# lh3/bfc

Hardware: AMD Instinct MI355X
Metric: M k-mers/s counted (bloom+htab) on 150 bp reads (higher is better)
Workload: dtype u64

## Files before the change

bfc_amd/_lib.py:

```python
import ctypes as C
import os

HERE = os.path.dirname(os.path.abspath(__file__))
SO = os.environ.get("BFC_GPU_LIB") or os.path.join(HERE, "libbfc_gpu.so")

u64p = C.POINTER(C.c_uint64)
u32p = C.POINTER(C.c_uint32)
f32p = C.POINTER(C.c_float)


class BfcOpt(C.Structure):
    _fields_ = [("chunk_size", C.c_int), ("n_threads", C.c_int), ("no_mt_io", C.c_int), ("q", C.c_int), ("k", C.c_int),
                ("filter_mode", C.c_int), ("refine_ec", C.c_int), ("no_qual", C.c_int), ("min_frac", C.c_float),
                ("l_pre", C.c_int), ("bf_shift", C.c_int), ("n_hashes", C.c_int), ("discard", C.c_int),
                ("max_end_ext", C.c_int), ("win_multi_ec", C.c_int), ("min_cov", C.c_int),
                ("w_ec", C.c_int), ("w_ec_high", C.c_int), ("w_absent", C.c_int), ("w_absent_high", C.c_int),
                ("max_path_diff", C.c_int), ("max_heap", C.c_int)]


class BfcBf(C.Structure):
    _fields_ = [("n_shift", C.c_int), ("n_hashes", C.c_int), ("b", C.POINTER(C.c_uint8))]


class BfcKmer(C.Structure):
# ... 41 lines not shown
    "bfcg_mg_scatter": (C.c_int, [C.c_void_p, C.c_void_p, C.c_void_p, C.c_uint64, C.c_void_p, u32p]),
    "bfcg_mg_process": (C.c_int, [C.c_void_p, C.c_void_p, u32p]),
    "bfcg_mg_allow_onepass": (None, [C.c_void_p, C.c_int]),
    "bfcg_group_unique_id": (C.c_int, [C.c_void_p]),
    "bfcg_group_create": (C.c_void_p, [C.POINTER(BfcgParams), C.c_int, C.c_int, C.c_int, C.POINTER(C.c_int), C.c_void_p, C.c_int]),
    "bfcg_group_destroy": (None, [C.c_void_p]),
    "bfcg_group_info": (C.c_int, [C.c_void_p, C.POINTER(C.c_int)]),
    "bfcg_group_slab_mode": (C.c_int, [C.c_void_p]),
    "bfcg_group_lazy_batches": (C.c_uint64, [C.c_void_p]),
    "bfcg_group_exchange_bytes": (C.c_int, [C.c_void_p, u64p]),
    "bfcg_group_ctx": (C.c_void_p, [C.c_void_p, C.c_int]),
    "bfcg_group_reset": (C.c_int, [C.c_void_p]),
    "bfcg_group_count_batch_dev": (C.c_int, [C.c_void_p, C.POINTER(C.c_void_p), C.POINTER(C.c_void_p), u64p]),
    "bfcg_group_count_batch_host": (C.c_int, [C.c_void_p, C.c_void_p, C.c_void_p, C.c_uint64]),
    "bfcg_group_sync": (C.c_int, [C.c_void_p]),
    "bfcg_group_stats": (C.c_int, [C.c_void_p, u64p]),
    "bfcg_group_progress": (C.c_int, [C.c_void_p, u64p, u64p, u64p, C.c_int]),
    "bfcg_group_export_table": (C.c_void_p, [C.c_void_p]),
    "bfcg_group_export_bloom": (C.POINTER(BfcBf), [C.c_void_p, C.c_int]),
    "bfcg_group_export_bloom_resident": (C.POINTER(BfcBf), [C.c_void_p, C.c_int]),
    "bfcg_trim_create": (C.c_void_p, [C.c_int, C.POINTER(BfcBf), C.c_int, C.c_uint64, C.c_uint64]),
    "bfcg_trim_destroy": (None, [C.c_void_p]),
    "bfcg_trim_batch": (C.c_int, [C.c_void_p, C.c_void_p, C.c_void_p, C.c_uint64, u64p, C.c_uint64, C.c_float, C.POINTER(C.c_int32), C.POINTER(C.c_int32)]),
    "bfcg_trim_last_ms": (C.c_float, [C.c_void_p]),
    "bfcg_trim_adopted": (C.c_int, [C.c_void_p]),
    "bfcg_trim_dev_seq": (C.c_void_p, [C.c_void_p]),
    "bfcg_stream_batches": (C.c_uint64, [C.c_void_p]),
    "bfc_ch_union": (C.c_void_p, [C.POINTER(C.c_void_p), C.c_int]),
    "bfc_ingest_digest": (C.c_int, [C.c_char_p, C.c_uint64, C.c_uint64, C.c_int, u64p]),
    "bfc_ingest_planes_digest": (C.c_int, [C.c_char_p, C.c_uint64, C.c_uint64, C.c_int, C.c_int, C.c_int, u64p]),
    "bfc_pgz_digest": (C.c_int, [C.c_char_p, C.c_int, C.c_uint64, C.c_uint64, u64p]),
    "bfcg_kcov_create": (C.c_void_p, [C.c_void_p, C.c_int, C.c_uint64]),
    "bfcg_kcov_attach": (C.c_void_p, [C.c_void_p, C.c_uint64]),
    "bfcg_kcov_destroy": (None, [C.c_void_p]),
    "bfcg_kcov_batch": (C.c_int, [C.c_void_p, C.c_void_p, C.c_void_p, C.c_uint64, C.c_int, C.c_void_p]),
    "bfcg_kcov_last_ms": (C.c_float, [C.c_void_p]),
    "bfcg_kcov_dev_seq": (C.c_void_p, [C.c_void_p]),
    "bfcg_kcov_dev_out": (C.c_void_p, [C.c_void_p]),
    "bfcg_dev_alloc": (C.c_void_p, [C.c_void_p, C.c_uint64]),
    "bfcg_dev_free": (None, [C.c_void_p, C.c_void_p]),
    "bfcg_h2d": (C.c_int, [C.c_void_p, C.c_void_p, C.c_void_p, C.c_uint64]),
    "bfcg_d2h": (C.c_int, [C.c_void_p, C.c_void_p, C.c_void_p, C.c_uint64]),
    "bfcg_host_alloc": (C.c_void_p, [C.c_uint64]),
    "bfcg_host_free": (None, [C.c_void_p]),
    "bfcg_stats": (C.c_int, [C.c_void_p, u64p]),
    "bfcg_progress": (C.c_int, [C.c_void_p, u64p, u64p, u64p, C.c_int]),
    "bfcg_partition_info": (C.c_int, [C.c_void_p, u64p]),
    "bfcg_s1wc_launches": (C.c_uint64, []),
    "bfcg_table_info": (C.c_int, [C.c_void_p, C.POINTER(C.c_int)]),
    "bfcg_last_batch_ms": (C.c_int, [C.c_void_p, f32p]),
    "bfcg_stage_ms": (C.c_int, [C.c_void_p, C.POINTER(C.c_double), u64p, C.c_int]),
    "bfcg_bloom_to_host": (C.c_int, [C.c_void_p, C.c_int, C.c_void_p]),
    "bfcg_export_bloom": (C.POINTER(BfcBf), [C.c_void_p, C.c_int]),
    "bfcg_export_bloom_resident": (C.POINTER(BfcBf), [C.c_void_p, C.c_int]),
    "bfcg_resident_drop": (None, [C.c_void_p]),
    "bfcg_export_table": (C.c_void_p, [C.c_void_p]),
    "bfcg_export_table_resident": (C.c_void_p, [C.c_void_p]),
    "bfc_ch_get_lpre": (C.c_int, [C.c_void_p]),
    "bfc_ch_export_sorted": (C.c_uint64, [C.c_void_p, u32p, u64p]),
    "bfcg_ec_create": (C.c_void_p, [C.c_void_p, C.POINTER(BfcOpt), C.c_int, C.c_uint64, C.c_uint64]),
    "bfcg_ec_attach": (C.c_void_p, [C.c_void_p, C.POINTER(BfcOpt), C.c_uint64, C.c_uint64]),
    "bfcg_ec_batch": (C.c_int, [C.c_void_p, C.c_void_p, C.c_void_p, C.c_uint64, u64p, C.c_uint64, u32p, u32p]),
    "bfcg_ec_destroy": (None, [C.c_void_p]),
    "bfcg_ec_last_ms": (C.c_float, [C.c_void_p]),
    "bfcg_ec_host_reads": (C.c_uint64, [C.c_void_p]),
    "bfcg_ec_last_lookups": (C.c_uint64, [C.c_void_p]),
    "bfcg_ec_retry_reads": (C.c_uint64, [C.c_void_p]),
    "bfcg_ec_adopted": (C.c_int, [C.c_void_p]),
    "bfcg_ec1_host": (C.c_int, [C.c_void_p, C.POINTER(BfcOpt), C.c_int, C.c_void_p, C.c_void_p, u32p, u32p]),
    "bfcg_ec_batch_refine": (C.c_int, [C.c_void_p, C.c_void_p, C.c_void_p, C.c_uint64, u64p, C.c_uint64, u32p, u32p, u32p, u32p]),
    "bfcg_ec1_host_refine": (C.c_int, [C.c_void_p, C.POINTER(BfcOpt), C.c_int, C.c_void_p, C.c_void_p, C.c_uint32, C.c_uint32, u32p, u32p]),
    "bfcg_ec_parse_stats": (C.c_int, [C.c_char_p, u32p, u32p]),
    "bfcg_kmers_create": (C.c_void_p, [C.c_void_p, C.c_int]),
    "bfcg_kmers_attach": (C.c_void_p, [C.c_void_p]),
    "bfcg_kmers_destroy": (None, [C.c_void_p]),
    "bfcg_kmers_info": (C.c_int, [C.c_void_p, C.POINTER(C.c_int)]),
    "bfcg_kmers_hist": (C.c_int, [C.c_void_p, u64p, u64p]),
    "bfcg_kmers_sub_sizes": (C.c_int, [C.c_void_p, u32p]),
    "bfcg_kmers_hist_sizes": (C.c_int, [C.c_void_p, u64p, u64p, u32p]),
    "bfcg_kmers_list": (C.c_int, [C.c_void_p, C.c_int, C.c_int, C.c_uint32, C.c_uint32, C.c_void_p, C.c_void_p, C.c_uint64, u64p]),
    "bfcg_kmers_last_ms": (C.c_float, [C.c_void_p]),
    "bfcg_kmer_decode_host": (C.c_int, [C.c_int, C.c_int, C.c_uint32, C.c_uint64, u64p]),
    "bfcg_kmer_2str": (None, [C.c_int, u64p, C.c_char_p]),
    "bfcg_kmers_format": (C.c_uint64, [C.c_int, C.c_void_p, C.c_void_p, C.c_uint64, C.c_void_p]),
    "bfcg_kmers_format_sizes": (C.c_uint64, [C.c_void_p, C.c_uint64, C.c_void_p]),
    "bfcg_kmers_lookup": (C.c_int, [C.c_void_p, C.c_void_p, C.c_uint64, C.c_void_p, u64p]),
    "bfcg_kmers_profile": (C.c_int, [C.c_void_p, C.c_void_p, C.c_void_p, C.c_uint64, C.c_void_p]),
    "bfcg_kmer_from_str": (C.c_int, [C.c_int, C.c_char_p, u64p]),
    "bfcg_kmer_occ_host": (C.c_int, [C.c_void_p, u64p]),
    "bfcg_kmers_occ_host": (None, [C.c_void_p, C.c_void_p, C.c_uint64, C.c_void_p]),
    "bfcg_kmers_parse": (C.c_uint64, [C.c_int, C.c_char_p, C.c_uint64, C.c_void_p, C.c_uint64, u64p]),
    "bfcg_lookup_format": (C.c_uint64, [C.c_char_p, C.c_uint64, C.c_void_p, C.c_uint64, C.c_void_p]),
    "bfcg_profile_format": (C.c_uint64, [C.c_void_p, C.c_uint64, C.c_void_p]),
    "bfcg_kmers_read_stats": (C.c_int, [C.c_void_p, C.c_void_p, C.c_void_p, C.c_uint64, C.c_void_p, C.c_uint64, C.c_int, C.c_void_p]),
    "bfcg_read_stats_host": (C.c_int, [C.c_void_p, C.c_void_p, C.c_uint64, C.c_void_p, C.c_uint64, C.c_int, C.c_void_p]),
    "bfcg_read_stats_format": (C.c_uint64, [C.c_void_p, C.c_uint64, C.c_void_p]),
    "bfcg_hash_positions": (C.c_int, [C.c_void_p, C.c_void_p, C.c_void_p, C.c_uint64, u64p]),
    "bfcg_seen_flags": (C.c_int, [C.c_void_p, C.c_void_p, C.c_uint64]),
}

_lib = None


def load():
    global _lib
    if _lib is None:
        if not os.path.exists(SO):
            raise OSError("libbfc_gpu.so is not built (run `python -m bfc_amd.build`); there is no fallback path")
        L = C.CDLL(SO)
        for name, (res, args) in SYMBOLS.items():
            f = getattr(L, name)
            f.restype = res
            f.argtypes = args
        _lib = L
    return _lib


def build_id():
    return load().bfcg_build_id().decode()


def check_build_id():
    from . import build
    have, want = build_id(), "src:" + build.source_hash()
    if not have.startswith(want):
        raise OSError("libbfc_gpu.so is stale: built from %s, the tree is %s (run `python -m bfc_amd.build`)" % (have, want))
    return have
```

bfc_amd/api.py:

```python
import ctypes as C
import math

import numpy as np

from . import _lib
from ._lib import BfcOpt, BfcgParams, BfcKmer, u64p, u32p, f32p

STAT_NAMES = {0: "n_kmers", 1: "n_high", 2: "n_seen", 3: "n_keys", 4: "tab_ovf", 5: "err_pool", 6: "slow_buckets", 7: "crowded_regions", 8: "tab_cshift", 9: "n_batches"}


class BfcGpuError(RuntimeError):
    pass


def bfc_opt_init():
    o = BfcOpt()
    o.chunk_size = 100000000
    o.n_threads = 1
    o.q = 20
    o.k = 33
    o.l_pre = 20
    o.bf_shift = 33
    o.n_hashes = 4
    o.min_frac = 0.9
# ... 217 lines not shown
        self = cls.__new__(cls)
        self.L = _lib.load()
        self.ctx, self.params, self._borrowed = ctx, params, True
        self.rank, self.n_ranks, self.bf_shift, self.k = 0, n_ranks, params.bf_shift, params.k
        return self

    def _ck(self, rc):
        if rc != 0:
            raise BfcGpuError(self.L.bfcg_last_error().decode())

    def close(self):
        if self.ctx and not getattr(self, "_borrowed", False):
            self.L.bfcg_destroy(self.ctx)
        self.ctx = None

    def __del__(self):
        try:
            self.close()
        except Exception:
            pass

    def reset(self):
        self._ck(self.L.bfcg_reset(self.ctx))

    def count_host(self, seq_stream, qual_stream=None):
        seq_stream = np.ascontiguousarray(seq_stream, dtype=np.uint8)
        q = np.ascontiguousarray(qual_stream, dtype=np.uint8) if qual_stream is not None else None
        self._ck(self.L.bfcg_count_batch_host(self.ctx, seq_stream.ctypes.data, q.ctypes.data if q is not None else None, len(seq_stream)))

    def count_planes(self, planes, first_pos, n_pos, has_qual=True):
        planes = np.ascontiguousarray(planes, dtype=np.uint32)
        assert planes.ndim == 2 and planes.shape[0] == 4
        self._ck(self.L.bfcg_count_batch_planes(self.ctx, planes.ctypes.data, planes.shape[1], first_pos, n_pos, 1 if has_qual else 0))

    def count_dev(self, d_seq, d_qual, n_pos):
        self._ck(self.L.bfcg_count_batch_dev(self.ctx, d_seq, d_qual, n_pos))

    def mg_info(self):
        out = (C.c_int * 4)()
        self.L.bfcg_mg_info(self.ctx, out)
        return dict(nb1=out[0], nb_loc=out[1], rec_bytes=out[2], n_ranks=out[3])

    def batch_limit(self):
        return int(self.L.bfcg_batch_limit(self.ctx))

    def mg_scatter(self, d_seq, d_qual, n_pos, d_send):
        counts = np.zeros(self.mg_info()["nb1"], dtype=np.uint32)
        self._ck(self.L.bfcg_mg_scatter(self.ctx, d_seq, d_qual, n_pos, d_send, counts.ctypes.data_as(u32p)))
        return counts

    def mg_process(self, d_recv, seg_cnt):
        seg_cnt = np.ascontiguousarray(seg_cnt, dtype=np.uint32)
        self._ck(self.L.bfcg_mg_process(self.ctx, d_recv, seg_cnt.ctypes.data_as(u32p)))

    def dev_alloc(self, nbytes):
        p = self.L.bfcg_dev_alloc(self.ctx, nbytes)
        if not p:
            raise BfcGpuError(self.L.bfcg_last_error().decode())
        return p

    def dev_free(self, p):
        self.L.bfcg_dev_free(self.ctx, p)

    def h2d(self, dptr, arr):
        arr = np.ascontiguousarray(arr)
        self._ck(self.L.bfcg_h2d(self.ctx, dptr, arr.ctypes.data, arr.nbytes))

    def sync(self):
        self._ck(self.L.bfcg_sync(self.ctx))

    def stats(self):
        out = np.zeros(16, dtype=np.uint64)
        self._ck(self.L.bfcg_stats(self.ctx, out.ctypes.data_as(u64p)))
        d = {STAT_NAMES[i]: int(out[i]) for i in STAT_NAMES}
        d["stream_batches"] = int(self.L.bfcg_stream_batches(self.ctx))
        d["phase_cycles"] = [int(out[i]) for i in range(10, 16)]
        return d

    def table_info(self):
        out = (C.c_int * 4)()
        self.L.bfcg_table_info(self.ctx, out)
        return dict(segments=bool(out[0]), seg_shift=out[1], tab_cshift=out[2], seg_growths=out[3])

    def partition_info(self):
        out = (C.c_uint64 * 2)()
        self.L.bfcg_partition_info(self.ctx, out)
        return dict(one_pass=bool(out[0] & 1), level2_one_pass=bool(out[0] & 2), replayed_batches=int(out[1]))

    def s1wc_launches(self):
        return int(self.L.bfcg_s1wc_launches())

    def last_batch_ms(self):
        out = np.zeros(6, dtype=np.float32)
        self.L.bfcg_last_batch_ms(self.ctx, out.ctypes.data_as(f32p))
        return dict(hist1=float(out[0]), scatter1=float(out[1]), level2=float(out[2]), bloom=float(out[3]), commit=float(out[4]), total=float(out[5]))

    def stage_ms(self, reset=False):
        out = (C.c_double * 6)()
        n = C.c_uint64()
        self._ck(self.L.bfcg_stage_ms(self.ctx, out, C.byref(n), int(reset)))
        return dict(hist1=out[0], scatter1=out[1], level2=out[2], bloom=out[3], commit=out[4], total=out[5]), int(n.value)

    def bloom_bytes(self, which=0):
        out = np.empty((1 << (self.bf_shift - 3)) // self.n_ranks, dtype=np.uint8)
        self._ck(self.L.bfcg_bloom_to_host(self.ctx, which, out.ctypes.data))
        return out

    def export_bloom(self, which=0, resident=False):
        p = (self.L.bfcg_export_bloom_resident if resident else self.L.bfcg_export_bloom)(self.ctx, which)
        if not p:
            raise BfcGpuError(self.L.bfcg_last_error().decode())
        return HostBloom(p)

    def export_table(self):
        p = self.L.bfcg_export_table(self.ctx)
        if not p:
            raise BfcGpuError(self.L.bfcg_last_error().decode())
        return HostTable(p)

    def hash_positions(self, seq_stream, qual_stream=None):
        seq_stream = np.ascontiguousarray(seq_stream, dtype=np.uint8)
        q = np.ascontiguousarray(qual_stream, dtype=np.uint8) if qual_stream is not None else None
        out = np.zeros((len(seq_stream), 3), dtype=np.uint64)
        self._ck(self.L.bfcg_hash_positions(self.ctx, seq_stream.ctypes.data, q.ctypes.data if q is not None else None, len(seq_stream), out.ctypes.data_as(u64p)))
        return out

    def seen_flags(self, n_pos):
        out = np.zeros(n_pos, dtype=np.uint8)
        self._ck(self.L.bfcg_seen_flags(self.ctx, out.ctypes.data, n_pos))
        return out


class GpuGroup:

    def __init__(self, k, bf_shift, devices, max_batch_pos, n_ranks=None, first_rank=0, uid=None, transport=0, q=20, n_hashes=4, l_pre=20,
                 filter_mode=0, track_order=False, table_layout=0, region_shift=0, tab_cshift=0):
        self.L = _lib.load()
        p = BfcgParams()
        self.L.bfcg_params_default(C.byref(p))
        p.k, p.q, p.bf_shift, p.n_hashes, p.l_pre, p.filter_mode = k, q, bf_shift, n_hashes, l_pre, filter_mode
        p.max_batch_pos, p.region_shift, p.tab_cshift, p.track_order, p.table_layout = int(max_batch_pos), region_shift, tab_cshift, int(track_order), int(table_layout)
        self.params, self.k, self.bf_shift = p, k, bf_shift
        self.devices = list(devices)
        self.n_local = len(self.devices)
        self.n_ranks = n_ranks if n_ranks is not None else self.n_local
        dv = (C.c_int * self.n_local)(*self.devices)
        self._uid = (C.c_uint8 * 128).from_buffer_copy(bytes(uid)) if uid is not None else None
        self.g = self.L.bfcg_group_create(C.byref(p), self.n_ranks, first_rank, self.n_local, dv, self._uid, transport)
        if not self.g:
            raise BfcGpuError("bfcg_group_create failed: " + self.L.bfcg_last_error().decode())

    @staticmethod
    def unique_id():
        L = _lib.load()
        buf = (C.c_uint8 * 128)()
        if L.bfcg_group_unique_id(buf) != 0:
            raise BfcGpuError(L.bfcg_last_error().decode())
        return bytes(buf)

    def _ck(self, rc):
        if rc != 0:
            raise BfcGpuError(self.L.bfcg_last_error().decode())

    def close(self):
        if self.g:
            self.L.bfcg_group_destroy(self.g)
            self.g = None

    def __del__(self):
        try:
# ... 417 lines not shown
```

bfc_amd/csrc/bfcg_bloom3.hip:

```cpp
#include <hip/hip_runtime.h>
#include <stdint.h>
#include <stdlib.h>
#include "kmer_dev.h"
#include "bfcg_internal.h"
#include "bfcg_dev.h"

using namespace bfcg;

#define B3_UND 0x40000000u
#define B3_SEEN 0x40000000u
#define B3_COLD_NR 8
template <int BT, int PF, bool COLD>
__global__ __launch_bounds__(BT, PF <= 2 ? 8 : 6) void k_bloom3(KParams P, BloomArgs A)
{
	extern __shared__ __attribute__((aligned(16))) unsigned char smem[];
	__shared__ uint32_t s_list_n, s_ovf, s_pool_off, s_emit_n, s_fs_used, s_wb_n, s_pad3[2];
	const uint32_t f = blockIdx.x;
	const bool ho_log = A.ho_stride != 0;
	if (batch_poisoned(A)) { if (ho_log && threadIdx.x == 0) A.ho_mark[f] = A.ho_cur[f]; return; }
	uint32_t rs, n;
	region_list(A, f, rs, n);
	if (n == 0) { if (threadIdx.x == 0) { if (ho_log) A.ho_mark[f] = A.ho_cur[f]; else if (A.agg_cnt) A.agg_cnt[f] = 0; } return; }
	uint32_t ho_cur0 = 0;
	unsigned long long *ho_base;
	if (ho_log) {
		ho_cur0 = A.ho_cur[f];
		if (ho_cur0 + n > A.ho_stride) {
			if (threadIdx.x == 0) { atomicAdd(&A.stats[(size_t)(f & (ST_SLOTS - 1)) * ST_N + ST_ERR_POOL], 1ULL); A.ho_mark[f] = ho_cur0; }
			return;
		}
		ho_base = A.ho + (uint64_t)f * A.ho_stride + ho_cur0;
	} else ho_base = reinterpret_cast<unsigned long long *>(A.stream_out) + rs;
	A.stats += (size_t)(f & (ST_SLOTS - 1)) * ST_N;
	const uint32_t region_dw = 16u << P.R;
	unsigned char *sp = smem;
	unsigned int *region = reinterpret_cast<unsigned int *>(sp); sp += (size_t)region_dw * 4;
	const uint32_t nblk = 1u << P.R;
	unsigned int *bcnt = reinterpret_cast<unsigned int *>(sp), *boff = bcnt + nblk;
	if (COLD) sp += (size_t)(2 * nblk + 4) * 4;
	unsigned int *fs = reinterpret_cast<unsigned int *>(sp); if (!COLD) sp += (size_t)P.fs_cap * 4;
	unsigned int *la = reinterpret_cast<unsigned int *>(sp); sp += (size_t)P.list_cap * 4;
	unsigned int *lb = reinterpret_cast<unsigned int *>(sp); sp += (size_t)P.list_cap * 4;
	unsigned short *lc = reinterpret_cast<unsigned short *>(sp); sp += (size_t)P.list_cap * 2;
	unsigned short *ord = reinterpret_cast<unsigned short *>(sp);
	const uint32_t fs_mask = P.fs_cap - 1;
	const uint32_t *recs = A.recs + (uint64_t)rs * 3;
	unsigned int *g_region = reinterpret_cast<unsigned int *>(A.bloom) + (uint64_t)f * region_dw;
	const uint32_t imp = (P.f_base + f) >> P.F2;
	const Dec3 D = dec3_geom(P);
	const int tid = threadIdx.x, lane = tid & 63;
	const uint32_t mask_a = (1u << D.a) - 1u, imp_sh = D.n ? imp << D.lo : 0u, sh_up = D.lo + D.n;
#ifdef BFCG_MEASURE
	const bool timing = BFCG_ABL(P, 64) && tid == 0;
	long long tq[7] = {0, 0, 0, 0, 0, 0, 0};
	if (timing) tq[0] = clock64();
#endif
	auto addr3 = [&](uint32_t d0, uint32_t d1) -> uint32_t {
		const uint32_t y0d = d0 & mask_a, upper = y0d >> D.up;
		const uint32_t y0lo = D.n ? (y0d & D.lowmask) | imp_sh | (upper << sh_up) : y0d;
		const uint32_t y1lo = __builtin_amdgcn_alignbit(d1, d0, D.a) & D.mk32;
		const uint32_t hh = upper | (((y0lo - y1lo) ^ y1lo) << D.sh_x);
		uint32_t h2 = (hh >> 9) & 511u;
		h2 |= (uint32_t)((h2 & 31u) == 0);
		return (y0d & D.rmask) | ((hh & 511u) << 8) | (h2 << 17);
	};
	auto entry3 = [&](uint32_t d0, uint32_t d1) -> unsigned long long {
		const unsigned long long AA = d0 | ((unsigned long long)d1 << 32);
		const unsigned long long y1 = (AA >> D.a) & ((1ULL << P.k) - 1);
		const uint32_t y0d = d0 & mask_a;
		const unsigned long long id = (unsigned long long)((y0d & D.rmask) | ((y0d >> D.up) << D.R)) | (y1 << D.sh_y1);
		return (id << 1) | (unsigned long long)((d1 >> D.sh_flag) & 1u);
	};
	RecW<3> cur[PF], nxt[PF];
#pragma unroll
	for (int u = 0; u < PF; ++u) {
		const uint32_t i = tid + u * BT;
		cur[u].d[0] = cur[u].d[1] = cur[u].d[2] = 0; nxt[u] = cur[u];
		if (i < n) cur[u] = rec_load<3>(recs + (uint64_t)i * 3);
		if (i + BT * PF < n) nxt[u] = rec_load<3>(recs + (uint64_t)(i + BT * PF) * 3);
	}
	{
		const uint4 *src = reinterpret_cast<const uint4 *>(g_region);
		uint4 *dst = reinterpret_cast<uint4 *>(region);
		for (uint32_t i = tid; i < region_dw / 4; i += BT) dst[i] = src[i];
		if constexpr (COLD) { for (uint32_t i = tid; i < 2 * nblk + 4; i += BT) bcnt[i] = 0; }
		else {
			uint4 *f4 = reinterpret_cast<uint4 *>(fs);
			for (uint32_t i = tid; i < P.fs_cap / 4; i += BT) f4[i] = make_uint4(FS32_EMPTY, FS32_EMPTY, FS32_EMPTY, FS32_EMPTY);
		}
		if (tid == 0) { s_list_n = 0; s_emit_n = 0; s_ovf = 0; s_fs_used = 0; s_wb_n = 0; }
	}
	__syncthreads();
#ifdef BFCG_MEASURE
	if (timing) tq[1] = clock64();
#endif
	volatile uint32_t *v_ovf = &s_ovf;

	for (uint32_t base = 0; base < n; base += BT * PF) {
		uint32_t pk[PF], um[PF];
#pragma unroll
		for (int u = 0; u < PF; ++u) {
			pk[u] = 0; um[u] = 0;
			if (base + u * BT + (uint32_t)(tid & ~63) < n) {
				pk[u] = addr3(cur[u].d[0], cur[u].d[1]);
				const B3Pos b = b3_positions((pk[u] >> 8) & 511u, pk[u] >> 17);
				const uint32_t bl64 = (pk[u] & 255u) << 6;
				const uint32_t w0 = *b3_wordp(region, bl64, b.b0), w1 = *b3_wordp(region, bl64, b.b1), w2 = *b3_wordp(region, bl64, b.b2), w3 = *b3_wordp(region, bl64, b.b3);
				um[u] = (b3_bit(w0, b.b0) | (b3_bit(w1, b.b1) << 1) | (b3_bit(w2, b.b2) << 2) | (b3_bit(w3, b.b3) << 3)) ^ 15u;
			}
		}
		unsigned long long ms[PF], ml[PF];
		uint32_t tot_s = 0, tot_l = 0;
#pragma unroll
		for (int u = 0; u < PF; ++u) {
			const bool act = base + tid + u * BT < n;
			ms[u] = __ballot(act && um[u] == 0); ml[u] = __ballot(act && um[u] != 0);
			tot_s += (uint32_t)__popcll(ms[u]); tot_l += (uint32_t)__popcll(ml[u]);
		}
		uint32_t o_s = 0, o_l = 0;
		if (lane == 0) { if (tot_s) o_s = atomicAdd(&s_emit_n, tot_s); if (tot_l) o_l = atomicAdd(&s_list_n, tot_l); }
		o_s = __builtin_amdgcn_readfirstlane(o_s); o_l = __builtin_amdgcn_readfirstlane(o_l);
#pragma unroll
		for (int u = 0; u < PF; ++u) {
			const uint32_t below_lo = (uint32_t)__builtin_amdgcn_mbcnt_lo((uint32_t)ms[u], 0u), below_s = (uint32_t)__builtin_amdgcn_mbcnt_hi((uint32_t)(ms[u] >> 32), below_lo);
			const uint32_t blow_lo = (uint32_t)__builtin_amdgcn_mbcnt_lo((uint32_t)ml[u], 0u), below_l = (uint32_t)__builtin_amdgcn_mbcnt_hi((uint32_t)(ml[u] >> 32), blow_lo);
			const bool act = base + tid + u * BT < n;
			if (act && um[u] == 0) {
				ho_base[o_s + below_s] = entry3(cur[u].d[0], cur[u].d[1]);
				if (A.seen_out) A.seen_out[cur[u].d[2]] = 2;
			} else if (act) {
				const uint32_t li = o_l + below_l;
				if (li < P.list_cap) {
					la[li] = cur[u].d[2]; lb[li] = pk[u] | (um[u] << 26); lc[li] = (unsigned short)(base + tid + u * BT);
					if constexpr (COLD) __hip_atomic_fetch_add(&bcnt[pk[u] & 255u], 1u, __ATOMIC_RELAXED, __HIP_MEMORY_SCOPE_WORKGROUP);
				}
			}
			o_s += (uint32_t)__popcll(ms[u]); o_l += (uint32_t)__popcll(ml[u]);
		}
		if (base + BT * PF < n) {
#pragma unroll
			for (int u = 0; u < PF; ++u) {
				cur[u] = nxt[u];
				const uint32_t i = base + 2 * BT * PF + tid + u * BT;
				if (i < n) nxt[u] = rec_load<3>(recs + (uint64_t)i * 3);
			}
		}
	}
	__syncthreads();
#ifdef BFCG_MEASURE
	if (timing) tq[2] = clock64();
#endif
	const uint32_t ln = s_list_n;
	const bool ovf_list = ln > P.list_cap || ln > (COLD ? (uint32_t)(B3_COLD_NR * BT) : 8191u) || n > 65535u;
	bool dirty = true;
	if constexpr (COLD) {
		if (!ovf_list) {
			if (tid < 64) {
				const uint32_t per = (nblk + 63u) >> 6, b0 = (uint32_t)tid * per;
				uint32_t v[4] = {0, 0, 0, 0}, sum = 0;
#pragma unroll
				for (int t = 0; t < 4; ++t) if ((uint32_t)t < per && b0 + t < nblk) { v[t] = bcnt[b0 + t]; sum += v[t]; }
				uint32_t inc = sum;
#pragma unroll
				for (int o = 1; o < 64; o <<= 1) { const uint32_t x = __shfl_up(inc, o); if (lane >= o) inc += x; }
				uint32_t run = inc - sum;
#pragma unroll
				for (int t = 0; t < 4; ++t) if ((uint32_t)t < per && b0 + t < nblk) { boff[b0 + t] = run; bcnt[b0 + t] = run; run += v[t]; }
				if (tid == 63) boff[nblk] = inc;
			}
			__syncthreads();
			for (uint32_t li = tid; li < ln; li += BT) ord[atomicAdd(&bcnt[lb[li] & 255u], 1u)] = (unsigned short)li;
			__syncthreads();
			uint32_t mv[B3_COLD_NR];
#pragma unroll
			for (int t = 0; t < B3_COLD_NR; ++t) {
				const uint32_t pos = (uint32_t)tid + (uint32_t)t * BT;
				mv[t] = 0;
				if (pos < ln) {
					const uint32_t li = ord[pos], x = la[li], bl = lb[li] & 255u, s0 = boff[bl], s1 = boff[bl + 1];
					uint32_t r = 0;
					for (uint32_t j = s0; j < s1; ++j) r += (uint32_t)(la[ord[j]] < x);
					mv[t] = ((s0 + r) << 16) | li;
				}
			}
			__syncthreads();
#pragma unroll
			for (int t = 0; t < B3_COLD_NR; ++t) { const uint32_t pos = (uint32_t)tid + (uint32_t)t * BT; if (pos < ln) ord[mv[t] >> 16] = (unsigned short)mv[t]; }
			__syncthreads();
			if ((uint32_t)tid < nblk) {
				const uint32_t bl = (uint32_t)tid, bl64 = bl << 6, s0 = boff[bl], s1 = boff[bl + 1];
				uint32_t li_n = s0 < s1 ? ord[s0] : 0u, w_n = s0 < s1 ? lb[li_n] : 0u;
				for (uint32_t j = s0; j < s1; ++j) {
					const uint32_t li = li_n, w = w_n;
					if (j + 1 < s1) { li_n = ord[j + 1]; w_n = lb[li_n]; }
					const B3Pos b = b3_positions((w >> 8) & 511u, (w >> 17) & 511u);
					unsigned int *p0 = b3_wordp(region, bl64, b.b0), *p1 = b3_wordp(region, bl64, b.b1), *p2 = b3_wordp(region, bl64, b.b2), *p3 = b3_wordp(region, bl64, b.b3);
					const uint32_t w0 = *p0, w1 = *p1, w2 = *p2, w3 = *p3;
					const uint32_t clr = (b3_bit(w0, b.b0) | (b3_bit(w1, b.b1) << 1) | (b3_bit(w2, b.b2) << 2) | (b3_bit(w3, b.b3) << 3)) ^ 15u;
					if (clr == 0) lb[li] = w | B3_SEEN;
					else {
						if (clr & 1u) __hip_atomic_fetch_or(p0, 1u << (b.b0 & 31u), __ATOMIC_RELAXED, __HIP_MEMORY_SCOPE_WORKGROUP);
						if (clr & 2u) __hip_atomic_fetch_or(p1, 1u << (b.b1 & 31u), __ATOMIC_RELAXED, __HIP_MEMORY_SCOPE_WORKGROUP);
						if (clr & 4u) __hip_atomic_fetch_or(p2, 1u << (b.b2 & 31u), __ATOMIC_RELAXED, __HIP_MEMORY_SCOPE_WORKGROUP);
						if (clr & 8u) __hip_atomic_fetch_or(p3, 1u << (b.b3 & 31u), __ATOMIC_RELAXED, __HIP_MEMORY_SCOPE_WORKGROUP);
					}
				}
			}
			__syncthreads();
			for (uint32_t t0 = 0; t0 < ln; t0 += BT) {
				const uint32_t li = t0 + tid;
				bool seen = false;
				if (li < ln) {
					seen = (lb[li] & B3_SEEN) != 0;
					if (A.seen_out) A.seen_out[la[li]] = seen ? 2 : 1;
				}
				const unsigned long long vote = __ballot(seen);
				if (vote) {
					uint32_t o = 0;
					if (lane == 0) o = atomicAdd(&s_emit_n, (uint32_t)__popcll(vote));
					o = __builtin_amdgcn_readfirstlane(o);
					if (seen) {
						const RecW<3> r = rec_load<3>(recs + (uint64_t)lc[li] * 3);
						ho_base[o + (uint32_t)__builtin_amdgcn_mbcnt_hi((uint32_t)(vote >> 32), __builtin_amdgcn_mbcnt_lo((uint32_t)vote, 0u))] = entry3(r.d[0], r.d[1]);
					}
				}
			}
			dirty = ln != 0;
			__syncthreads();
		}
	} else
	if (!ovf_list) {
		for (uint32_t li = tid; li < ln; li += BT) {
			const uint32_t w = lb[li], bl = w & 255u, bl64 = bl << 6, um = (w >> 26) & 15u;
			const B3Pos b = b3_positions((w >> 8) & 511u, (w >> 17) & 511u);
			uint32_t o0 = 0, o1 = 0, o2 = 0, o3 = 0;
			if (um & 1u) o0 = atomicOr(b3_wordp(region, bl64, b.b0), 1u << (b.b0 & 31u));
			if (um & 2u) o1 = atomicOr(b3_wordp(region, bl64, b.b1), 1u << (b.b1 & 31u));
			if (um & 4u) o2 = atomicOr(b3_wordp(region, bl64, b.b2), 1u << (b.b2 & 31u));
			if (um & 8u) o3 = atomicOr(b3_wordp(region, bl64, b.b3), 1u << (b.b3 & 31u));
			uint32_t cm = (b3_bit(o0, b.b0) | (b3_bit(o1, b.b1) << 1) | (b3_bit(o2, b.b2) << 2) | (b3_bit(o3, b.b3) << 3)) & um;
			if (cm) {
				*(volatile uint32_t *)&s_fs_used = 1;
				__hip_atomic_fetch_or(&region[bl * 16u], 1u, __ATOMIC_RELAXED, __HIP_MEMORY_SCOPE_WORKGROUP);
				const uint32_t idx = la[li];
				const uint32_t p01 = b.b0 | (b.b1 << 16), p23 = b.b2 | (b.b3 << 16);
				while (cm) {
					const int j = __ffs((int)cm) - 1;
					cm &= cm - 1;
					const uint32_t bj = ((j & 2 ? p23 : p01) >> ((j & 1) << 4)) & 0xffffu;
					if (!fs32_insert(fs, fs_mask, bl * 512u + bj, li, idx, la)) *v_ovf = 1;
				}
			}
		}
	}
	__syncthreads();
#ifdef BFCG_MEASURE
	if (timing) tq[6] = clock64();
#endif
	const bool ovf = ovf_list || s_ovf;
	if (COLD && !ovf) ;
	else if (!ovf) {
		if (s_fs_used) {
			auto compete_entry = [&](uint32_t li) {
				const uint32_t w = lb[li], bl = w & 255u, um = (w >> 26) & 15u;
				const B3Pos b = b3_positions((w >> 8) & 511u, (w >> 17) & 511u);
				const uint32_t q0 = bl * 512u + b.b0, q1 = bl * 512u + b.b1, q2 = bl * 512u + b.b2, q3 = bl * 512u + b.b3;
				const uint32_t c0 = fs[fs32_slot(q0, fs_mask)], c1 = fs[fs32_slot(q1, fs_mask)], c2 = fs[fs32_slot(q2, fs_mask)], c3 = fs[fs32_slot(q3, fs_mask)];
				uint32_t todo = ((uint32_t)(c0 != FS32_EMPTY) | ((uint32_t)(c1 != FS32_EMPTY) << 1) | ((uint32_t)(c2 != FS32_EMPTY) << 2) | ((uint32_t)(c3 != FS32_EMPTY) << 3)) & um;
				bool und = todo == um;
				if (todo) {
					const uint32_t idx = la[li];
					const uint32_t p01 = b.b0 | (b.b1 << 16), p23 = b.b2 | (b.b3 << 16);
					while (todo) {
						const int j = __ffs((int)todo) - 1;
						todo &= todo - 1;
						const uint32_t bj = ((j & 2 ? p23 : p01) >> ((j & 1) << 4)) & 0xffffu;
						und &= fs32_compete(fs, fs_mask, bl * 512u + bj, li, idx, la);
					}
				}
				if (und) lb[li] = w | B3_UND;
			};
			unsigned short *const wb = lc + ln;
			const uint32_t wb_cap = P.list_cap - ln;
			for (uint32_t li0 = 0; li0 < ln; li0 += BT) {
				const uint32_t li = li0 + tid;
				bool want = false;
				if (li < ln) {
					want = (region[(lb[li] & 255u) * 16u] & 1u) != 0;
					if (!want && A.seen_out) A.seen_out[la[li]] = 1;
				}
				const unsigned long long vote = __ballot(want);
				if (vote) {
					uint32_t o = 0;
					if (lane == 0) o = atomicAdd(&s_wb_n, (uint32_t)__popcll(vote));
					o = __builtin_amdgcn_readfirstlane(o);
					if (want) {
						const uint32_t slot = o + (uint32_t)__builtin_amdgcn_mbcnt_hi((uint32_t)(vote >> 32), __builtin_amdgcn_mbcnt_lo((uint32_t)vote, 0u));
						if (slot < wb_cap) wb[slot] = (unsigned short)li;
						else compete_entry(li);
					}
				}
			}
			__syncthreads();
			const uint32_t wb_all = s_wb_n, wb_n = wb_all < wb_cap ? wb_all : wb_cap;
			for (uint32_t t = tid; t < wb_n; t += BT) compete_entry(wb[t]);
			__syncthreads();
			const bool wl_ok = wb_all <= wb_cap;
			const uint32_t cn = wl_ok ? wb_n : ln;
			for (uint32_t t0 = 0; t0 < cn; t0 += BT) {
				const uint32_t t = t0 + tid;
				uint32_t li = 0;
				bool seen = false;
				if (t < cn) {
					li = wl_ok ? (uint32_t)wb[t] : t;
					const uint32_t w = lb[li];
					if (w & B3_UND) {
						const uint32_t bl = w & 255u, um = (w >> 26) & 15u;
						const B3Pos b = b3_positions((w >> 8) & 511u, (w >> 17) & 511u);
						bool first = false;
						if (um & 1u) first |= fs32_lookup(fs, fs_mask, bl * 512u + b.b0) == li;
						if (um & 2u) first |= fs32_lookup(fs, fs_mask, bl * 512u + b.b1) == li;
						if (um & 4u) first |= fs32_lookup(fs, fs_mask, bl * 512u + b.b2) == li;
						if (um & 8u) first |= fs32_lookup(fs, fs_mask, bl * 512u + b.b3) == li;
						seen = !first;
					}
					if (A.seen_out) A.seen_out[la[li]] = seen ? 2 : 1;
				}
				const unsigned long long vote = __ballot(seen);
				if (vote) {
					uint32_t o = 0;
					if (lane == 0) o = atomicAdd(&s_emit_n, (uint32_t)__popcll(vote));
					o = __builtin_amdgcn_readfirstlane(o);
					if (seen) {
						const RecW<3> r = rec_load<3>(recs + (uint64_t)lc[li] * 3);
						ho_base[o + (uint32_t)__popcll(vote & ((1ULL << lane) - 1))] = entry3(r.d[0], r.d[1]);
					}
				}
			}
			for (uint32_t i = tid; i < (1u << P.R); i += BT) region[i * 16u] &= ~0xffu;
		} else if (A.seen_out) {
			for (uint32_t li = tid; li < ln; li += BT) A.seen_out[la[li]] = 1;
		}
		dirty = ln != 0;
		__syncthreads();
	} else {
		const int nh = 4;
		uint64_t want = (uint64_t)n * nh * 2;
		const uint64_t lim = (uint64_t)(1u << P.R) * 512 * 2;
		if (want > lim) want = lim;
		uint32_t cap = 1024; while (cap < want) cap <<= 1;
		if (tid == 0) {
			uint32_t sl = f & (A.pool_slices - 1);
			while (atomicCAS(&A.pool[sl], 0ULL, 1ULL) != 0ULL) sl = (sl + 1) & (A.pool_slices - 1);
			s_pool_off = sl; s_emit_n = 0;
			atomicAdd(&A.stats[ST_SLOW_BUCKETS], 1ULL);
		}
		{
			const uint4 *src = reinterpret_cast<const uint4 *>(g_region);
			uint4 *dst = reinterpret_cast<uint4 *>(region);
			for (uint32_t i = tid; i < region_dw / 4; i += BT) dst[i] = src[i];
		}
		__syncthreads();
		unsigned long long *gfs = A.pool + A.pool_slices + (uint64_t)s_pool_off * lim;
		for (uint32_t i = tid; i < cap; i += BT) gfs[i] = FS_EMPTY;
		__threadfence();
		__syncthreads();
		const uint32_t gmask = cap - 1;
		for (uint32_t i = tid; i < n; i += BT) {
			const RecW<3> r = rec_load<3>(recs + (uint64_t)i * 3);
			const uint32_t w = addr3(r.d[0], r.d[1]), bl = w & 255u;
			uint32_t z = (w >> 8) & 511u;
			for (int j = 0; j < nh; ++j) {
				const uint32_t b = bloom_next(z, w >> 17);
				if (!b3_bit(*b3_wordp(region, bl << 6, b), b)) fs_insert<true>(gfs, gmask, bl * 512 + b, r.d[2], gmask);
			}
		}
		__threadfence();
		__syncthreads();
		for (uint32_t i0 = 0; i0 < n; i0 += BT) {
			const uint32_t i = i0 + tid;
			bool seen = false;
			RecW<3> r; r.d[0] = r.d[1] = r.d[2] = 0;
			if (i < n) {
				r = rec_load<3>(recs + (uint64_t)i * 3);
				const uint32_t w = addr3(r.d[0], r.d[1]), bl = w & 255u;
				uint32_t z = (w >> 8) & 511u; bool first = false, unresolved = false;
				for (int j = 0; j < nh; ++j) {
					uint32_t b = bloom_next(z, w >> 17), fi;
					if (fs_lookup<true>(gfs, gmask, bl * 512 + b, fi)) {
						unresolved = true; first |= (fi == r.d[2]);
						atomicOr(b3_wordp(region, bl << 6, b), 1u << (b & 31));
					}
				}
				seen = !unresolved || !first;
				if (A.seen_out) A.seen_out[r.d[2]] = seen ? 2 : 1;
			}
			const unsigned long long vote = __ballot(seen);
			if (vote) {
				uint32_t o = 0;
				if (lane == 0) o = atomicAdd(&s_emit_n, (uint32_t)__popcll(vote));
				o = __builtin_amdgcn_readfirstlane(o);
				if (seen) ho_base[o + (uint32_t)__popcll(vote & ((1ULL << lane) - 1))] = entry3(r.d[0], r.d[1]);
			}
		}
		__syncthreads();
		if (tid == 0) { __threadfence(); atomicExch(&A.pool[s_pool_off], 0ULL); }
	}
#ifdef BFCG_MEASURE
	if (timing) tq[3] = clock64();
#endif
	if (dirty) {
		uint4 *dst = reinterpret_cast<uint4 *>(g_region);
		const uint4 *src = reinterpret_cast<const uint4 *>(region);
		for (uint32_t i = tid; i < region_dw / 4; i += BT) dst[i] = src[i];
	}
#ifdef BFCG_MEASURE
	if (timing) tq[4] = clock64();
#endif
	if (tid == 0) {
		const uint32_t ns = s_emit_n;
		if (ns) atomicAdd(&A.stats[ST_SEEN], (unsigned long long)ns);
		if (ho_log) { A.ho_cur[f] = ho_cur0 + ns; A.ho_mark[f] = ho_cur0 + ns; }
		else if (A.agg_cnt) A.agg_cnt[f] = ns;
	}
#ifdef BFCG_MEASURE
	if (timing) {
		tq[5] = clock64();
		for (int t = 0; t < 5; ++t) atomicAdd(&A.stats[10 + t], (unsigned long long)(tq[t + 1] - tq[t]));
		atomicAdd(&A.stats[15], (unsigned long long)(tq[6] - tq[2]));
	}
#endif
	(void)s_pad3;
}

namespace bfcg {

typedef void (*BloomFn)(KParams, BloomArgs);
static BloomFn bloom3_kernel(bool pf2, bool cold)
{
	if (cold) return pf2 ? k_bloom3<512, 2, true> : k_bloom3<512, 4, true>;
	return pf2 ? k_bloom3<512, 2, false> : k_bloom3<512, 4, false>;
}
static hipError_t set_bloom3_max_lds(BloomFn fn, int lds) { return hipFuncSetAttribute((const void *)fn, hipFuncAttributeMaxDynamicSharedMemorySize, lds < BLOOM3_LDS_FLOOR ? BLOOM3_LDS_FLOOR : lds); }
hipError_t set_bloom3_lds_attr(int lds)
{
	hipError_t e = hipSuccess;
	for (int i = 0; i < 4 && e == hipSuccess; ++i) e = set_bloom3_max_lds(bloom3_kernel(i & 1, i & 2), lds);
	return e;
}

void run_bloom3(const KParams &P, const BloomArgs &A, int nfine, size_t lds, hipStream_t st)
{
	static int pf = 0;
	if (!pf) { const char *e = getenv("BFCG_B3_PF"); pf = e && atoi(e) == 2 ? 2 : e && atoi(e) == 4 ? 4 : 1; }
	const bool pf2 = P.b3_cold ? P.b3_warm != 0 : pf == 2 || (pf == 1 && P.b3_warm);
	hipLaunchKernelGGL(bloom3_kernel(pf2, P.b3_cold != 0), dim3(nfine), dim3(512), lds, st, P, A);
}

}

struct Dec4 { int up, iw, is; uint32_t rmask; };
__device__ __forceinline__ Dec4 dec4_geom(const KParams &P)
{
	Dec4 g;
	g.up = P.rec_n ? P.rec_lo : P.bf_shift - 9;
	const int io = (P.k - P.rec_n) + P.k + 1;
	g.iw = io >> 5; g.is = io & 31; g.rmask = (1u << P.R) - 1u;
	return g;
}
template <int BT, int PF>
__global__ __launch_bounds__(BT, 6) void k_bloom3fm(KParams P, BloomArgs A)
{
	extern __shared__ __attribute__((aligned(16))) unsigned char smem[];
	__shared__ uint32_t s_list_n, s_seen;
	const uint32_t f = blockIdx.x;
	if (batch_poisoned(A)) return;
	uint32_t rs, n;
	region_list(A, f, rs, n);
	if (n == 0) return;
	A.stats += (size_t)(f & (ST_SLOTS - 1)) * ST_N;
	const uint32_t region_dw = 16u << P.R, nblk = 1u << P.R;
	unsigned char *sp = smem;
	unsigned int *region = reinterpret_cast<unsigned int *>(sp); sp += (size_t)region_dw * 4;
	unsigned int *region_hi = reinterpret_cast<unsigned int *>(sp); sp += (size_t)region_dw * 4;
	unsigned int *bcnt = reinterpret_cast<unsigned int *>(sp), *boff = bcnt + nblk; sp += (size_t)(2 * nblk + 4) * 4;
	unsigned int *la = reinterpret_cast<unsigned int *>(sp); sp += (size_t)P.list_cap * 4;
	unsigned int *lb = reinterpret_cast<unsigned int *>(sp); sp += (size_t)P.list_cap * 4;
	unsigned short *ord = reinterpret_cast<unsigned short *>(sp);
	const uint32_t *recs = A.recs + (uint64_t)rs * 4;
	unsigned int *g_region = reinterpret_cast<unsigned int *>(A.bloom) + (uint64_t)f * region_dw;
	unsigned int *g_region_hi = reinterpret_cast<unsigned int *>(A.bloom_hi) + (uint64_t)f * region_dw;
	const Dec4 D = dec4_geom(P);
	const int tid = threadIdx.x, lane = tid & 63;
	auto addr4 = [&](uint32_t d0, uint32_t d1) -> uint32_t {
		const uint32_t hh = __builtin_amdgcn_alignbit(d1, d0, D.up);
		uint32_t h2 = (hh >> 9) & 511u;
		h2 |= (uint32_t)((h2 & 31u) == 0);
		return (d0 & D.rmask) | ((hh & 511u) << 8) | (h2 << 17);
	};
	auto idx4 = [&](const RecW<4> &r) -> uint32_t {
		const uint32_t a = D.iw == 0 ? r.d[0] : D.iw == 1 ? r.d[1] : D.iw == 2 ? r.d[2] : r.d[3], b = D.iw == 0 ? r.d[1] : D.iw == 1 ? r.d[2] : r.d[3];
		return D.is ? __builtin_amdgcn_alignbit(b, a, D.is) : a;
	};
	auto set_hi = [&](uint32_t bl64, const B3Pos &b) {
		__hip_atomic_fetch_or(b3_wordp(region_hi, bl64, b.b0), 1u << (b.b0 & 31u), __ATOMIC_RELAXED, __HIP_MEMORY_SCOPE_WORKGROUP);
		__hip_atomic_fetch_or(b3_wordp(region_hi, bl64, b.b1), 1u << (b.b1 & 31u), __ATOMIC_RELAXED, __HIP_MEMORY_SCOPE_WORKGROUP);
		__hip_atomic_fetch_or(b3_wordp(region_hi, bl64, b.b2), 1u << (b.b2 & 31u), __ATOMIC_RELAXED, __HIP_MEMORY_SCOPE_WORKGROUP);
		__hip_atomic_fetch_or(b3_wordp(region_hi, bl64, b.b3), 1u << (b.b3 & 31u), __ATOMIC_RELAXED, __HIP_MEMORY_SCOPE_WORKGROUP);
	};
	{
		const uint4 *src = reinterpret_cast<const uint4 *>(g_region), *src2 = reinterpret_cast<const uint4 *>(g_region_hi);
		uint4 *dst = reinterpret_cast<uint4 *>(region), *dst2 = reinterpret_cast<uint4 *>(region_hi);
		for (uint32_t i = tid; i < region_dw / 4; i += BT) { dst[i] = src[i]; dst2[i] = src2[i]; }
	}
	uint32_t r = 0, sh = 32, seen_total = 0;
	bool dirty = false;
	const uint32_t cap = P.list_cap < (uint32_t)(B3_COLD_NR * BT) ? P.list_cap : (uint32_t)(B3_COLD_NR * BT);
	for (;;) {
		for (uint32_t i = tid; i < 2 * nblk + 4; i += BT) bcnt[i] = 0;
		if (tid == 0) { s_list_n = 0; s_seen = 0; }
		__syncthreads();
		uint32_t my_seen = 0;
		RecW<4> rec[PF], nxt[PF];
#pragma unroll
		for (int u = 0; u < PF; ++u) {
			const uint32_t i = tid + u * BT;
			rec[u].d[0] = rec[u].d[1] = rec[u].d[2] = rec[u].d[3] = 0; nxt[u] = rec[u];
			if (i < n) rec[u] = rec_load<4>(recs + (uint64_t)i * 4);
			if (i + BT * PF < n) nxt[u] = rec_load<4>(recs + (uint64_t)(i + BT * PF) * 4);
		}
		for (uint32_t base = 0; base < n; base += BT * PF) {
			uint32_t pk[PF], um[PF], ix[PF];
			bool act[PF];
#pragma unroll
			for (int u = 0; u < PF; ++u) {
				ix[u] = idx4(rec[u]);
				act[u] = base + tid + u * BT < n && (sh == 32 || (ix[u] >> sh) == r);
				pk[u] = addr4(rec[u].d[0], rec[u].d[1]);
				const B3Pos b = b3_positions((pk[u] >> 8) & 511u, pk[u] >> 17);
// ... 132 lines not shown
```

bfc_amd/csrc/bfcg_ctx.hip:

```cpp
#include <hip/hip_runtime.h>
#include <stdint.h>
#include <stdio.h>
#include <stdlib.h>
#include <string.h>
#include <stdarg.h>
#include <sys/mman.h>
#include <time.h>
#include <vector>
#include <thread>
#include "bfc_gpu.h"
#include "bfcg_internal.h"
#include "bfc_host.h"

using namespace bfcg;

static thread_local char g_err[512] = "";
enum { HO_MAX_PAGES = BFCG_HO_MAX_PAGES };
enum { OP_FLAG_WORDS = 12, OP_STICKY = 8 };
static double dbg_now(void) { struct timespec ts; clock_gettime(CLOCK_MONOTONIC, &ts); return ts.tv_sec + 1e-9 * ts.tv_nsec; }
static inline void set_seg_shift(KParams &P, int s, int blk_max) { P.seg_shift = s; P.seg_blk = s < blk_max ? s : blk_max; }
int bfcg::fail(const char *fmt, ...)
{
	va_list ap; va_start(ap, fmt); vsnprintf(g_err, sizeof(g_err), fmt, ap); va_end(ap);
	fprintf(stderr, "[E::bfcg] %s\n", g_err);
	return -1;
}

struct bfcg_ctx {
	bfcg_params_t prm;
	KParams P;
	BatchBufs B;
	hipStream_t st;
	hipStream_t stA;
	hipStream_t stC;
	hipEvent_t evt[2][7];
	hipEvent_t evA[2], evB[2], evCopy;
	uint32_t *rows1[2], *chunk1[2], *start1[2]; uint64_t *recs1[2];
	uint8_t *d_seq2[2], *d_qual2[2];
	uint32_t *d_planes[2];
	uint64_t plane_cap;
	int cur, pend;
	int used[2];
	uint8_t *d_seq, *d_qual;
	unsigned long long *h_stats;
	unsigned long long *h_snap[2];
	uint64_t call_no, slot_call[2];
	int call_depth;
	uint64_t final_call, call_keys[64];
	uint64_t n_batches;
	float last_ms[6];
	double sum_ms[6]; uint64_t n_timed;
	int rw;
	uint64_t bloom_bytes;
	int n_ranks, rank, log2n;
	uint32_t *d_seg, *h_seg;
	size_t seg_words;
	uint64_t recv_cap;
	uint64_t keys_last, grow[2];
	uint64_t crowded_last;
	int stream_mode;
	uint32_t *stream_out; uint64_t n_stream_batches;
	double seen_per_pos;
	int cold;
	uint64_t seen_last, pos_final, slot_pos[2];
	int pipeline;
	int seg_ok;
	int seg_total_max;
	int seg_blk_max;
	int b3_ok;
	uint32_t fs_cap_w, list_cap_w;
	uint32_t list_cap_cw;
	uint32_t list_cap_c;
	int seg_init_shift;
	int seg_escaped;
	uint64_t n_seg_grow;
	int onepass_ok, onepass;
	uint32_t *op_cursor[2], *op_seg[2], *op_flags, *h_flags[2];
	int unfinished, unfinished_mg;
	uint32_t *h_rows[2]; int rows_slot;
	uint32_t op_cap; uint64_t op_min_pos;
	uint32_t *cnt2; uint32_t cap2; uint64_t recs2_n;
	struct opq_t { const uint8_t *seq, *qual; uint64_t n_pos; int slot; const void *recv; int mg; } opq[4]; int n_opq;
	int mg_op2_ok, mg_op2, mg_op2_allowed; uint32_t *mg_seg[4];
	int mg_slab_ok; int mg_seg_slab[4];
	uint64_t n_replayed;
	int reused;
	int seg_no_grow;
	int seg_cap_shift;
	unsigned long long *ho, *ho_keys, *h_ho_keys[2]; uint32_t *ho_cur, *ho_mark; uint32_t ho_stride; int ho_K;
	int ho_pending;
	uint64_t ho_page_call[HO_MAX_PAGES];
	int slot_commit[2]; uint64_t slot_page_call[2][HO_MAX_PAGES];
	int slot_all_committed[2];
	uint64_t keys_known;
	int commit_absorbed;
	uint64_t keys_per_batch; int n_commits, ho_window;
	unsigned long long *seg_spare; int seg_spare_shift;
};

extern "C" const char *bfcg_last_error(void) { return g_err; }
extern "C" void bfcg_set_error(const char *msg) { fail("%s", msg); }

extern "C" int bfcg_device_count(void)
{
	int ndev = 0;
	if (hipGetDeviceCount(&ndev) != hipSuccess) { (void)hipGetLastError(); return 0; }
	return ndev;
}

extern "C" void bfcg_params_default(bfcg_params_t *p)
{
	memset(p, 0, sizeof(*p));
	p->k = 33; p->q = 20; p->bf_shift = 33; p->n_hashes = 4; p->l_pre = 20;
	p->max_batch_pos = 1ULL << 27;
}

static int clamp_lpre(int k, int l_pre)
{
	if (k * 2 - l_pre > BFC_CH_KEYBITS) l_pre = k * 2 - BFC_CH_KEYBITS;
	if (l_pre > BFC_CH_MAXPRE) l_pre = BFC_CH_MAXPRE;
	return l_pre;
}

extern "C" bfcg_ctx_t *bfcg_create(const bfcg_params_t *prm)
{
	int ndev = 0;
	const bool timing = getenv("BFC_GPU_TIMING") != 0;
	const double t_c0 = dbg_now();
	if (hipGetDeviceCount(&ndev) != hipSuccess || ndev == 0) { fail("no HIP device available: the counting path has no CPU fallback"); return NULL; }
	const double t_c1 = dbg_now();
	if (prm->device < 0 || prm->device >= ndev) { fail("device %d out of range (%d devices)", prm->device, ndev); return NULL; }
	if (prm->k < 1 || prm->k > 63) { fail("k=%d outside [1,63] (bfc.h:8, htab.c:23)", prm->k); return NULL; }
	if (prm->bf_shift < 9 + 0 || prm->bf_shift > 37) { fail("bf_shift=%d outside [9,37] (bbf.c:9, bfc.h:9)", prm->bf_shift); return NULL; }
	if (prm->n_hashes < 1 || prm->n_hashes > 12) { fail("n_hashes=%d outside [1,12]", prm->n_hashes); return NULL; }
	if (prm->max_batch_pos == 0 || prm->max_batch_pos >= (1ULL << 32)) { fail("max_batch_pos must be in [1, 2^32)"); return NULL; }
	const int n_ranks = prm->n_ranks > 0 ? prm->n_ranks : 1;
	int log2n = 0; while ((1 << log2n) < n_ranks) ++log2n;
	if ((1 << log2n) != n_ranks || n_ranks > 64 || prm->rank < 0 || prm->rank >= n_ranks) { fail("n_ranks=%d must be a power of two <= 64 and 0 <= rank=%d < n_ranks", n_ranks, prm->rank); return NULL; }
	if (n_ranks > 1 && prm->max_batch_pos >= (1ULL << (32 - log2n))) { fail("with %d ranks a batch holds < 2^%d positions", n_ranks, 32 - log2n); return NULL; }
	BFCG_CKN((void)0, hipSetDevice(prm->device));

	bfcg_ctx_t *c = (bfcg_ctx_t *)calloc(1, sizeof(bfcg_ctx_t));
	if (!c) { fail("out of host memory"); return NULL; }
	c->prm = *prm;
	KParams &P = c->P;
	P.k = prm->k; P.q = prm->q; P.bf_shift = prm->bf_shift; P.n_hashes = prm->n_hashes; P.filter_mode = prm->filter_mode;
	P.l_pre = clamp_lpre(prm->k, prm->l_pre);
	if (!prm->filter_mode && 2 * prm->k < P.l_pre) {
		fail("k=%d is too small for l_pre=%d: the count table needs 2k >= l_pre (htab.c:45-58)", prm->k, P.l_pre); bfcg_destroy(c); return NULL;
	}
	{
		const char *e;
		P.R = prm->region_shift > 0 ? prm->region_shift : ((e = getenv("BFCG_R")) ? atoi(e) : 8);
		if (P.R > 10) P.R = 10;
		if (P.R < 4) P.R = 4;
		if (P.R > P.bf_shift - 9) P.R = P.bf_shift - 9;
		while (P.bf_shift - 9 - P.R > 20 && P.R < 10) ++P.R;
		P.F = P.bf_shift - 9 - P.R;
		if (P.F <= 8) { P.F1 = P.F; P.F2 = 0; }
		else { P.F2 = (P.F + 1) / 2; if (P.F2 > 10) P.F2 = 10; P.F1 = P.F - P.F2; }
		if (P.F2 > 0 && (e = getenv("BFCG_F1"))) {
			const int f1 = atoi(e);
			if (f1 >= 1 && f1 <= 10 && P.F - f1 >= 1 && P.F - f1 <= 10 && f1 >= log2n) { P.F1 = f1; P.F2 = P.F - f1; }
		}
		if (P.F1 > 10) { fail("bf_shift=%d needs more than two scatter levels at region_shift=%d", P.bf_shift, P.R); bfcg_destroy(c); return NULL; }
		if (n_ranks > 1 && P.F2 == 0) {
			if (P.F <= log2n) { fail("bf_shift=%d gives %d bloom regions: too few for %d ranks", P.bf_shift, 1 << P.F, n_ranks); bfcg_destroy(c); return NULL; }
			P.F1 = (P.F + 1) / 2 > log2n ? (P.F + 1) / 2 : log2n; P.F2 = P.F - P.F1;
// ... 524 lines not shown
static int seg_maintain(bfcg_ctx_t *c)
{
	KParams &P = c->P; BatchBufs &B = c->B;
	const uint64_t nf = nfine(c);
	const double t_dbg = dbg_now();
	struct dbg_guard { double t; int s0; const int *s1; ~dbg_guard() { if (getenv("BFCG_DEBUG") && *s1 != s0) fprintf(stderr, "[D::seg_maintain] shift %d -> %d: %.3f ms\n", s0, *s1, (dbg_now() - t) * 1e3); } } dg{t_dbg, P.seg_shift, &P.seg_shift};
	for (;;) {
		const uint64_t ovf = c->h_stats[ST_TAB_OVF];
		const int target = seg_target_shift(c);
		if (ovf == 0 && target == P.seg_shift) return 0;
		if (ovf > B.tab_ovf_cap) return fail("count table overflow list exhausted (%llu parked k-mers)", (unsigned long long)ovf);
		{
			size_t free_b = 0, total_b = 0;
			const bool no_room = hipMemGetInfo(&free_b, &total_b) == hipSuccess && ((nf << target) * 8) + (1ULL << 30) > (uint64_t)free_b + (c->seg_spare && c->seg_spare_shift >= target ? (nf << c->seg_spare_shift) * 8 : 0);
			if (no_room || target > c->seg_total_max) {
				if (ovf == 0 && (double)c->h_stats[ST_KEYS] < 0.85 * (double)(nf << P.seg_shift)) { c->seg_no_grow = 1; return 0; }
				if (target > c->seg_total_max) return seg_to_legacy(c);
				if (seg_to_legacy(c) == 0) return 0;
				return fail("count table of %llu keys cannot grow to 2^%d slots per region: %.1f GiB of device memory free", (unsigned long long)c->h_stats[ST_KEYS], target, free_b / 1073741824.0);
			}
		}
		const int old_shift = P.seg_shift, old_blk = P.seg_blk;
		unsigned long long *nt = 0;
		int nt_shift = target;
		set_seg_shift(P, target, c->seg_blk_max);
		if (c->seg_spare && c->seg_spare_shift >= target) { nt = c->seg_spare; nt_shift = c->seg_spare_shift; c->seg_spare = 0; }
		else {
			if (c->seg_spare) { BFCG_CK(hipFree(c->seg_spare)); c->seg_spare = 0; }
			BFCG_CK(hipMalloc(&nt, (nf << target) * 8));
		}
		run_seg_rehash(P, B.seg_tab, old_shift, old_blk, nt, (uint32_t)nf, c->st);
		BFCG_CK(hipStreamSynchronize(c->st));
		BFCG_CK(hipGetLastError());
		if (((nf << nt_shift) * 8) <= (16ULL << 30)) {
			if (c->seg_cap_shift < nt_shift && c->reused) { BFCG_CK(hipFree(B.seg_tab)); c->seg_spare = 0; if (hipMalloc(&c->seg_spare, (nf << nt_shift) * 8) != hipSuccess) { (void)hipGetLastError(); c->seg_spare = 0; } c->seg_spare_shift = nt_shift; }
			else { c->seg_spare = B.seg_tab; c->seg_spare_shift = c->seg_cap_shift; }
		} else BFCG_CK(hipFree(B.seg_tab));
		B.seg_tab = nt; c->seg_cap_shift = nt_shift;
		++c->n_seg_grow;
		if (ovf) {
			uint64_t *tmp = 0;
			BFCG_CK(hipMalloc(&tmp, ovf * 40));
			BFCG_CK(hipMemcpyAsync(tmp, B.tab_ovf, ovf * 40, hipMemcpyDeviceToDevice, c->st));
			BFCG_CK(hipMemsetAsync(&B.stats[(size_t)ST_SLOTS * ST_N], 0, 8, c->st));
			run_seg_replay(P, B.seg_tab, tmp, ovf, B.stats, B.tab_ovf, B.tab_ovf_cap, c->st);
			if (fetch_stats(c) != 0) return -1;
			BFCG_CK(hipFree(tmp));
		} else c->h_stats[ST_TAB_OVF] = 0;
	}
}

static int seg_to_legacy(bfcg_ctx_t *c, int for_export)
{
	KParams &P = c->P; BatchBufs &B = c->B;
	const uint64_t nf = nfine(c);
	const uint64_t keys = c->h_stats[ST_KEYS];
	if (c->seg_spare) { BFCG_CK(hipFree(c->seg_spare)); c->seg_spare = 0; }
	if (!for_export && !P.filter_mode && !B.agg_out) BFCG_CK(hipMalloc(&B.agg_out, nf * P.ag_cap * (P.track ? 32 : 24)));
	int cs = c->prm.tab_cshift > 0 ? c->prm.tab_cshift : 2;
	const uint64_t want = for_export ? keys + keys * 3 / 4 : 2 * keys + (c->prm.max_batch_pos / 4);
	while ((1ULL << (P.l_pre + cs)) < want && P.l_pre + cs < 36) ++cs;
	{
		size_t free_b = 0, total_b = 0;
		if (hipMemGetInfo(&free_b, &total_b) == hipSuccess)
			while (cs > 1 && (8ULL << (P.l_pre + cs)) + (2ULL << 30) > (uint64_t)free_b) --cs;
	}
	P.tab_cshift = cs;
	BFCG_CK(hipMalloc(&B.table, 8ULL << (P.l_pre + cs)));
	BFCG_CK(hipMemsetAsync(B.table, 0, 8ULL << (P.l_pre + cs), c->st));
	BFCG_CK(hipMemset2DAsync(B.stats + ST_KEYS, sizeof(unsigned long long) * ST_N, 0, sizeof(unsigned long long), ST_SLOTS, c->st));
	run_seg_to_table(P, B.seg_tab, (uint32_t)nf, B.table, B.stats, B.tab_ovf, B.tab_ovf_cap, c->st);
	BFCG_CK(hipStreamSynchronize(c->st));
	BFCG_CK(hipGetLastError());
	BFCG_CK(hipFree(B.seg_tab));
	B.seg_tab = 0;
	P.seg = 0; P.b3 = 0; c->seg_escaped = 1;
	BFCG_CK(set_bloom_lds_attr(P));
	if (fetch_stats(c) != 0) return -1;
	c->keys_last = c->h_stats[ST_KEYS];
	if (for_export && c->h_stats[ST_TAB_OVF] == 0) return 0;
	return table_maintain(c);
}

extern "C" int bfcg_partition_info(bfcg_ctx_t *c, uint64_t out[2]) { out[0] = (uint64_t)((c->onepass ? 1 : 0) | ((c->onepass || (c->mg_op2 && c->mg_op2_allowed)) && c->cap2 ? 2 : 0)); out[1] = c->n_replayed; return 0; }
extern "C" void bfcg_mg_allow_onepass(bfcg_ctx_t *c, int on) { c->mg_op2_allowed = on != 0; }

extern "C" int bfcg_table_info(bfcg_ctx_t *c, int out[4])
{
	out[0] = c->P.seg; out[1] = c->P.seg ? c->P.seg_shift : 0; out[2] = c->P.seg ? 0 : c->P.tab_cshift; out[3] = (int)c->n_seg_grow;
	return 0;
}


static KParams batch_params(const bfcg_ctx_t *c, int no_kstats, int onepass1)
{
	KParams Pt = c->P;
	Pt.no_kstats = no_kstats;
	Pt.dedupe = dedupe_hint(c);
	warm_tables(c, Pt);
	if (onepass1) {
		const char *e = getenv("BFCG_L2_BIG");
		const int want = e ? atoi(e) : 0;
		Pt.l2_big = c->cap2 && want > 0 && Pt.F2 >= (want == 1 ? 9 : 10) && scatter2_big_ok(Pt);
	}
	return Pt;
}

static int batch_bufs(bfcg_ctx_t *c, BatchBufs &Bt)
{
	if (ensure_agg(c) != 0 || use_stream(c) != 0) return -1;
	Bt = c->B;
	Bt.batch_hi = (unsigned long long)(c->n_batches + 1) << 32;
	Bt.stream = c->stream_mode; Bt.stream_out = c->stream_out;
	return 0;
}

struct StageB {
	const uint64_t *in1; const uint32_t *seg_beg, *seg_end; int n_seg, segs_per_bucket; const uint32_t *row_base, *bucket_start; uint64_t rec_bound;
	int slabs;
	int queued;
	uint64_t call, pos;
	const uint8_t *seq, *qual;
	const void *recv; const uint32_t *sizes; int sizes_slab;
	int finalise;
};

static int opq_push(bfcg_ctx_t *c, int b, const StageB &w)
{
	if (c->n_opq == 4) return fail("internal: one-pass queue overflow");
	int mg = 0;
	if (w.recv) {
		const size_t words = (size_t)c->n_ranks * (size_t)((1 << c->P.F1) >> c->log2n) * (w.sizes_slab ? 8 : 1);
		for (;; ++mg) { int used = 0; for (int i = 0; i < c->n_opq; ++i) used |= c->opq[i].mg == mg + 1; if (!used) break; }
		if (w.sizes) memcpy(c->mg_seg[mg], w.sizes, sizeof(uint32_t) * words); else memset(c->mg_seg[mg], 0, sizeof(uint32_t) * words);
		c->mg_seg_slab[mg++] = w.sizes_slab;
	}
	c->opq[c->n_opq++] = bfcg_ctx::opq_t{w.seq, w.qual, w.pos, b, w.recv, mg};
	return 0;
}

static int enqueue_stage_b(bfcg_ctx_t *c, int b, BatchBufs &Bt, const KParams &Pt, const StageB &w)
{
	if (handover_begin(c, Bt, b, w.slabs, w.call) != 0) return -1;
	run_stage_b(Pt, Bt, w.in1, w.seg_beg, w.seg_end, w.n_seg, w.segs_per_bucket, w.row_base, w.bucket_start, w.rec_bound, c->st, c->evt[b]);
	if (handover_end(c, Bt, b) != 0) return -1;
	if (w.queued) {
		BFCG_CK(hipMemcpyAsync(c->h_flags[b] + 1, c->op_flags + OP_STICKY, sizeof(uint32_t), hipMemcpyDeviceToHost, c->st));
		if (opq_push(c, b, w) != 0) return -1;
	}
	BFCG_CK(hipMemcpyAsync(c->h_snap[b], c->B.stats, sizeof(unsigned long long) * ST_N * (ST_SLOTS + 1), hipMemcpyDeviceToHost, c->st));
	c->slot_call[b] = c->call_no = w.call; c->slot_pos[b] = w.pos;
	BFCG_CK(hipEventRecord(c->evB[b], c->st));
	BFCG_CK(hipGetLastError());
	c->used[b] = 1;
	++c->n_batches;
	return w.finalise ? finalise_previous(c, b) : 0;
}

static int mg_stage_b(bfcg_ctx_t *c, int b, const void *d_recv, const uint32_t *d, int n_seg, int spb, uint64_t rec_bound, const uint32_t *sizes, int sizes_slab, int finalise)
{
	BatchBufs Bt;
	if (batch_bufs(c, Bt) != 0) return -1;
	const int op2_run = c->mg_op2 && c->mg_op2_allowed && c->cap2;
	const int op2 = op2_run && rec_bound >= 8 * nfine(c);
	if (op2_run) Bt.op_sticky = c->op_flags + OP_STICKY;
	if (op2) {
		Bt.cnt2 = c->cnt2; Bt.cap2 = c->cap2; Bt.op_flags = c->op_flags + 4 * b;
		BFCG_CK(hipMemsetAsync(Bt.op_flags, 0, 4 * sizeof(uint32_t), c->st));
	}
	const StageB w = {(const uint64_t *)d_recv, d, d + n_seg, n_seg, spb, d + 2 * n_seg, d + 3 * n_seg + 1, rec_bound, op2, op2_run, c->call_no + 1, rec_bound, nullptr, nullptr, d_recv, sizes, sizes_slab, finalise};
	return enqueue_stage_b(c, b, Bt, batch_params(c, 0, 0), w);
}


extern "C" int bfcg_mg_info(bfcg_ctx_t *c, int out[4])
{
	out[0] = 1 << c->P.F1; out[1] = (1 << c->P.F1) >> c->log2n; out[2] = c->rw; out[3] = c->n_ranks;
	return 0;
}

static int mg_scatter2(bfcg_ctx_t *c, const uint8_t *d_seq, const uint8_t *d_qual, uint64_t n_pos, void *d_send, uint32_t *counts, int no_kstats);
extern "C" int bfcg_mg_scatter(bfcg_ctx_t *c, const uint8_t *d_seq, const uint8_t *d_qual, uint64_t n_pos, void *d_send, uint32_t *counts) { return mg_scatter2(c, d_seq, d_qual, n_pos, d_send, counts, 0); }
extern "C" int bfcg_mg_scatter_again(bfcg_ctx_t *c, const uint8_t *d_seq, const uint8_t *d_qual, uint64_t n_pos, void *d_send, uint32_t *counts) { return mg_scatter2(c, d_seq, d_qual, n_pos, d_send, counts, 1); }
static inline hipStream_t mg_stage_a_stream(bfcg_ctx_t *c) { return c->n_ranks == 1 && !c->pipeline ? c->st : c->stA; }
static int mg_stage_a_begin(bfcg_ctx_t *c, int b, hipStream_t sA, const uint8_t *d_seq, const uint8_t **d_qual, uint64_t n_pos)
{
	if (batch_fits(c, n_pos) != 0) return -1;
	BFCG_CK(hipSetDevice(c->prm.device));
	if (n_pos == 0) {
		for (int i = 0; i < 3; ++i) BFCG_CK(hipEventRecord(c->evt[b][i], sA));
		return 1;
	}
	return same_block_offset(c, b, d_seq, d_qual, n_pos, sA);
}
static BatchBufs mg_slab_bufs(const bfcg_ctx_t *c, int b, uint32_t own_delta)
{
	const uint32_t nb_loc = (1u << c->P.F1) >> c->log2n;
	BatchBufs Bt = c->B;
	Bt.op_cursor = c->op_cursor[b]; Bt.op_seg = c->op_seg[b]; Bt.op_flags = c->op_flags + 4 * b; Bt.op_cap = c->op_cap; Bt.cap2 = c->cap2;
	Bt.op_own_lo = (uint32_t)c->rank * nb_loc; Bt.op_own_n = nb_loc; Bt.op_own_delta = own_delta;
	return Bt;
}
static int mg_scatter2(bfcg_ctx_t *c, const uint8_t *d_seq, const uint8_t *d_qual, uint64_t n_pos, void *d_send, uint32_t *counts, int no_kstats)
{
	const int nb1 = 1 << c->P.F1, b = c->cur;
	const hipStream_t sA = mg_stage_a_stream(c);
	const int begun = mg_stage_a_begin(c, b, sA, d_seq, &d_qual, n_pos);
	if (begun == 1) memset(counts, 0, sizeof(uint32_t) * nb1);
	if (begun) return begun < 0 ? -1 : 0;
	BatchBufs Bt = c->B;
	Bt.rows1 = c->rows1[b]; Bt.chunk1 = c->chunk1[b]; Bt.start1 = c->start1[b]; Bt.row_base = Bt.start1 + nb1 + 1;
	KParams Pa = c->P;
	Pa.no_kstats = no_kstats;
	run_stage_a(Pa, Bt, d_seq, d_qual, (int64_t)n_pos, (uint64_t *)d_send, sA, c->evt[b]);
	BFCG_CK(hipGetLastError());
	uint32_t *tmp = (uint32_t *)malloc(sizeof(uint32_t) * (nb1 + 1));
	hipError_t e = hipMemcpyAsync(tmp, Bt.start1, sizeof(uint32_t) * (nb1 + 1), hipMemcpyDeviceToHost, sA);
	if (e == hipSuccess) e = hipStreamSynchronize(sA);
	if (e != hipSuccess) { free(tmp); return fail("reading the level-1 bucket starts failed: %s", hipGetErrorString(e)); }
	for (int i = 0; i < nb1; ++i) counts[i] = tmp[i + 1] - tmp[i];
	free(tmp);
	return 0;
}

extern "C" int bfcg_mg_slab_info(bfcg_ctx_t *c, uint32_t out[2]) { out[0] = c->op_cap; out[1] = (uint32_t)(c->mg_slab_ok && c->op_cursor[0] != 0); return 0; }
extern "C" int bfcg_mg_scatter_slabs(bfcg_ctx_t *c, const uint8_t *d_seq, const uint8_t *d_qual, uint64_t n_pos, void *d_send, uint32_t own_delta, uint32_t *fills, int *overflow)
// ... 648 lines not shown
```

bfc_amd/csrc/bfcg_dev.h:

```cpp
#pragma once
#include <hip/hip_runtime.h>
#include <stdint.h>
#include "kmer_dev.h"
#include "bfcg_internal.h"

using namespace bfcg;

template <int RD> struct RecW { uint32_t d[RD]; };

template <int RD> __device__ __forceinline__ RecW<RD> rec_load(const uint32_t *p);
template <> __device__ __forceinline__ RecW<3> rec_load<3>(const uint32_t *p)
{ const uint3 v = *reinterpret_cast<const uint3 *>(p); RecW<3> r; r.d[0] = v.x; r.d[1] = v.y; r.d[2] = v.z; return r; }
template <> __device__ __forceinline__ RecW<4> rec_load<4>(const uint32_t *p)
{ const uint4 v = *reinterpret_cast<const uint4 *>(p); RecW<4> r; r.d[0] = v.x; r.d[1] = v.y; r.d[2] = v.z; r.d[3] = v.w; return r; }
template <> __device__ __forceinline__ RecW<5> rec_load<5>(const uint32_t *p)
{ RecW<5> r; r.d[0] = p[0]; r.d[1] = p[1]; r.d[2] = p[2]; r.d[3] = p[3]; r.d[4] = p[4]; return r; }
template <int RD> __device__ __forceinline__ void rec_store(uint32_t *p, const RecW<RD> &r);
template <> __device__ __forceinline__ void rec_store<3>(uint32_t *p, const RecW<3> &r)
{ *reinterpret_cast<uint3 *>(p) = make_uint3(r.d[0], r.d[1], r.d[2]); }
template <> __device__ __forceinline__ void rec_store<4>(uint32_t *p, const RecW<4> &r)
{ *reinterpret_cast<uint4 *>(p) = make_uint4(r.d[0], r.d[1], r.d[2], r.d[3]); }
template <> __device__ __forceinline__ void rec_store<5>(uint32_t *p, const RecW<5> &r)
{ p[0] = r.d[0]; p[1] = r.d[1]; p[2] = r.d[2]; p[3] = r.d[3]; p[4] = r.d[4]; }


struct TabOrder {
	unsigned long long *first, *sub_last;
	__device__ __forceinline__ void note(uint32_t sub, uint64_t slot, unsigned long long sf, unsigned long long sl) const
	{
		if (first) { atomicMin(&first[slot], sf); atomicMax(&sub_last[sub], sl); }
	}
};


#define FS_EMPTY 0xffffffffffffffffULL

template <bool GLOBAL>
__device__ __forceinline__ bool fs_insert(unsigned long long *tab, uint32_t cap_mask, uint32_t bitoff, uint32_t idx, uint32_t max_probe)
{
	const unsigned long long e = ((unsigned long long)bitoff << 32) | idx;
	uint32_t p = ((bitoff * 0x9E3779B1u) >> 12 ^ bitoff) & cap_mask;
	for (uint32_t probe = 0; probe <= max_probe; ++probe, p = (p + 1) & cap_mask) {
		unsigned long long cur = GLOBAL ? __hip_atomic_load(&tab[p], __ATOMIC_RELAXED, __HIP_MEMORY_SCOPE_AGENT) : tab[p];
		if (cur == FS_EMPTY) {
			cur = atomicCAS(&tab[p], FS_EMPTY, e);
			if (cur == FS_EMPTY) return true;
		}
		if ((uint32_t)(cur >> 32) == bitoff) { if (e < cur) atomicMin(&tab[p], e); return true; }
	}
	return false;
}
template <bool GLOBAL>
__device__ __forceinline__ bool fs_lookup(const unsigned long long *tab, uint32_t cap_mask, uint32_t bitoff, uint32_t &first)
{
	uint32_t p = ((bitoff * 0x9E3779B1u) >> 12 ^ bitoff) & cap_mask;
	for (uint32_t probe = 0; probe <= cap_mask; ++probe, p = (p + 1) & cap_mask) {
		unsigned long long cur = GLOBAL ? __hip_atomic_load((unsigned long long *)&tab[p], __ATOMIC_RELAXED, __HIP_MEMORY_SCOPE_AGENT) : tab[p];
		if (cur == FS_EMPTY) return false;
		if ((uint32_t)(cur >> 32) == bitoff) { first = (uint32_t)cur; return true; }
	}
	return false;
}

struct BloomArgs {
	const uint32_t *recs;
	const uint32_t *start;
	unsigned long long *bloom;
	unsigned long long *bloom_hi;
	unsigned long long *table;
	unsigned long long *stats;
	uint64_t *tab_ovf; uint32_t tab_ovf_cap; unsigned long long *ovf_cnt;
	unsigned long long *pool; uint32_t pool_slices;
	uint8_t *seen_out;
	uint64_t *agg_out;
	uint32_t *agg_cnt;
	uint32_t *stream_out;
	unsigned long long *seg_tab;
	uint32_t n_fine;
	TabOrder ord;
	unsigned long long batch_hi;
	const uint32_t *cnt2; uint32_t cap2;
	unsigned long long *ho; uint32_t ho_stride; uint32_t *ho_cur; uint32_t *ho_mark;
	uint32_t ho_pages, ho_mark_stride;
	unsigned long long *ho_keys;
	const uint32_t *flags;
	const uint32_t *sticky;
};

__device__ __forceinline__ void region_list(const BloomArgs &A, uint32_t f, uint32_t &rs, uint32_t &n)
{
	if (A.cap2) { const uint32_t c = A.cnt2[f]; rs = f * A.cap2; n = c < A.cap2 ? c : A.cap2; }
	else if (A.cnt2) { rs = A.start[f]; n = A.cnt2[f]; }
	else { rs = A.start[f]; n = A.start[f + 1] - rs; }
}
__device__ __forceinline__ bool batch_poisoned(const BloomArgs &A) { return (A.sticky && *A.sticky) || (A.flags && (A.flags[0] | A.flags[2])); }


struct Dec3 { int ok, a, lo, n, up, sh_x, R, sh_flag, sh_y1; uint32_t lowmask, rmask, mk32; };
__device__ __forceinline__ Dec3 dec3_geom(const KParams &P)
{
	Dec3 g;
	g.a = P.k - P.rec_n; g.lo = P.rec_lo; g.n = P.rec_n; g.up = P.rec_n ? P.rec_lo : P.bf_shift - 9; g.sh_x = P.k - (P.bf_shift - 9);
	g.R = P.R; g.sh_flag = g.a + P.k - 32; g.sh_y1 = P.k - P.F;
	g.lowmask = P.rec_n ? (1u << (P.rec_lo & 31)) - 1u : 0xffffffffu; g.rmask = (1u << P.R) - 1u; g.mk32 = P.k >= 32 ? 0xffffffffu : (1u << P.k) - 1u;
	g.ok = P.k >= P.bf_shift - 9 && P.bf_shift + 9 <= 2 * P.k && g.a >= 1 && g.a <= 31 && g.a + P.k >= 32 && (P.rec_n == 0 || P.rec_lo + P.rec_n <= 31)
	       && g.up <= g.a && g.sh_x >= 0 && g.sh_x <= 31 && g.sh_y1 >= 0 && g.sh_y1 <= 32 && (P.rec_n == 0 || P.rec_lo + P.rec_n == P.bf_shift - 9) && P.R <= g.up;
	return g;
}

#define FS32_EMPTY 0xffffffffu
__device__ __forceinline__ uint32_t fs32_slot(uint32_t bitoff, uint32_t mask) { return ((bitoff * 0x9E3779B1u) >> 12 ^ bitoff) & mask; }

__device__ __forceinline__ bool fs32_insert(unsigned int *fs, uint32_t mask, uint32_t bitoff, uint32_t li, uint32_t idx, const unsigned int *list_idx)
{
	const uint32_t e = (bitoff << 13) | li;
	uint32_t p = fs32_slot(bitoff, mask);
	for (int probe = 0; probe < 1024; ++probe, p = (p + 1) & mask) {
		uint32_t cur = fs[p];
		if (cur == FS32_EMPTY) {
			cur = atomicCAS(&fs[p], FS32_EMPTY, e);
			if (cur == FS32_EMPTY) return true;
		}
		if ((cur >> 13) == bitoff) {
			while (list_idx[cur & 0x1fffu] > idx) {
				uint32_t old = atomicCAS(&fs[p], cur, e);
				if (old == cur) break;
				cur = old;
			}
			return true;
		}
	}
	return false;
}
__device__ __forceinline__ bool fs32_compete(unsigned int *fs, uint32_t mask, uint32_t bitoff, uint32_t li, uint32_t idx, const unsigned int *list_idx)
{
	const uint32_t e = (bitoff << 13) | li;
	uint32_t p = fs32_slot(bitoff, mask);
	for (uint32_t probe = 0; probe <= mask; ++probe, p = (p + 1) & mask) {
		uint32_t cur = fs[p];
		if (cur == FS32_EMPTY) return false;
		if ((cur >> 13) == bitoff) {
			while (list_idx[cur & 0x1fffu] > idx) {
				uint32_t old = atomicCAS(&fs[p], cur, e);
				if (old == cur) break;
				cur = old;
			}
			return true;
		}
	}
	return false;
}
__device__ __forceinline__ uint32_t fs32_lookup(const unsigned int *fs, uint32_t mask, uint32_t bitoff)
{
	uint32_t p = fs32_slot(bitoff, mask);
	for (uint32_t probe = 0; probe <= mask; ++probe, p = (p + 1) & mask) {
		uint32_t cur = fs[p];
		if (cur == FS32_EMPTY) return FS32_EMPTY;
		if ((cur >> 13) == bitoff) return cur & 0x1fffu;
	}
	return FS32_EMPTY;
}


struct B3Pos { uint32_t b0, b1, b2, b3; };
__device__ __forceinline__ B3Pos b3_positions(uint32_t h1, uint32_t h2)
{
	const uint32_t u1 = h1 + h2, u2 = u1 + h2, u3 = u2 + h2, u4 = u3 + h2;
	const uint32_t c0 = h1, c1 = u1 & 511u, c2 = u2 & 511u, c3 = u3 & 511u, c4 = u4 & 511u;
	const bool s0 = c0 < 8u, s1 = s0 | (c1 < 8u), s2 = s1 | (c2 < 8u), s3 = s2 | (c3 < 8u);
	B3Pos p;
	p.b0 = s0 ? c1 : c0; p.b1 = s1 ? c2 : c1; p.b2 = s2 ? c3 : c2; p.b3 = s3 ? c4 : c3;
	if (__builtin_expect(min(min(p.b0, p.b1), min(p.b2, p.b3)) < 8u, 0)) {
		uint32_t z = h1;
		p.b0 = bloom_next(z, h2); p.b1 = bloom_next(z, h2); p.b2 = bloom_next(z, h2); p.b3 = bloom_next(z, h2);
	}
	return p;
}
__device__ __forceinline__ unsigned int *b3_wordp(unsigned int *region, uint32_t bl64, uint32_t b)
{ return reinterpret_cast<unsigned int *>(reinterpret_cast<unsigned char *>(region) + (bl64 | ((b >> 3) & 0x3cu))); }
__device__ __forceinline__ uint32_t b3_bit(uint32_t w, uint32_t b) { return __builtin_amdgcn_ubfe(w, b, 1u); }


namespace bfcg {
constexpr int BLOOM3_LDS_FLOOR = (53000 + 15) & ~15;
hipError_t set_bloom3_lds_attr(int lds);
void run_bloom3(const KParams &P, const BloomArgs &A, int nfine, size_t lds, hipStream_t st);
hipError_t set_bloom3fm_lds_attr(int lds);
void run_bloom3fm(const KParams &P, const BloomArgs &A, int nfine, size_t lds, hipStream_t st);
}
```

bfc_amd/csrc/bfcg_internal.h:

```cpp
#pragma once
#include <hip/hip_runtime.h>
#define BFCG_TILE1 4096
#define BFCG_BT1 256
#define BFCG_SCAN_CH 64
static inline int bfcg_rec_dwords(int k, int rec_n) { const int bits = 2 * k - rec_n + 33; return bits <= 96 ? 3 : bits <= 128 ? 4 : 5; }
static constexpr int bfcg_tile_of_rw(int rw) { return rw == 5 ? 2048 : rw == 4 ? 3072 : 4096; }
static constexpr int bfcg_tile1_of_rw(int rw) { return rw == 3 ? 4096 : 3072; }
#define BFCG_MAXB 1024
#define BFCG_HO_MAX_PAGES 8
#ifdef BFCG_MEASURE
#define BFCG_ABL(P, bits) ((P).ablate & (bits))
#else
#define BFCG_ABL(P, bits) 0
#endif
#include <stdint.h>
struct bfcg_ctx; struct bfcg_kcov;

struct bfcg_kmers {
	int k, l_pre, cshift, device, owns_table;
	hipStream_t st;
	hipEvent_t e0, e1;
	const unsigned long long *table;
	unsigned long long *d_hist;
	uint32_t *d_sizes;
	uint32_t *d_cnt; unsigned long long *d_off; uint64_t blk_cap;
	ulonglong2 *d_y; uint16_t *d_ch; uint64_t out_cap;
	ulonglong2 *d_qy; int16_t *d_qout; uint64_t q_cap;
	uint8_t *d_pseq; uint64_t pseq_cap; int16_t *d_pout; uint64_t pout_cap;
	unsigned long long *d_roff; uint64_t roff_cap; int32_t *d_rout; uint64_t rout_cap;
	float last_ms;
};

namespace bfcg {
#define BFCG_LOCAL __attribute__((visibility("hidden")))

enum { ST_KMERS = 0, ST_HIGH, ST_SEEN, ST_KEYS, ST_TAB_OVF, ST_ERR_POOL, ST_SLOW_BUCKETS, ST_CROWDED , ST_N = 16 };
enum { ST_SLOTS = 256 };

struct KParams {
	int k, q, bf_shift, n_hashes, l_pre, filter_mode;
	int R;
	int F, F1, F2;
	int tab_cshift;
	uint32_t fs_cap, list_cap;
	uint32_t ag_cap;
	uint32_t idx_rank;
	int track;
	int ablate;
	int bloom_bt;
	int seg;
	int seg_shift;
	int seg_blk;
	int seg_lo, seg_hi;
	uint32_t f_base;
	int no_kstats;
	int dedupe;
	uint32_t ct_cap;
	int rec_lo, rec_n;
	int b3;
	int b3_warm;
	int b3fm;
	int l2_big;
	int b3_cold;
};

struct BatchBufs {
	uint32_t *rows1, *chunk1;
	uint32_t *start1, *row_base;
	uint32_t *rows2, *start2;
	uint64_t *recs1, *recs2;
	uint64_t max_kmers;
	unsigned long long *bloom, *bloom_hi, *table;
	unsigned long long *stats;
	uint64_t *tab_ovf; uint32_t tab_ovf_cap;
	unsigned long long *pool; uint32_t pool_slices;
	uint8_t *seen_out;
	uint64_t *agg_out; uint32_t *agg_cnt;
	uint32_t *stream_out; int stream;
	uint32_t *op_cursor, *op_flags, *op_sticky, *op_seg; uint32_t op_cap;
	uint32_t op_own_lo, op_own_n, op_own_delta;
	uint32_t *cnt2; uint32_t cap2;
	uint32_t *cnt_live;
	unsigned long long *ho; uint32_t ho_stride; uint32_t *ho_cur, *ho_mark; uint32_t ho_mark_stride, ho_page; int ho_commit; unsigned long long *ho_keys;
	unsigned long long *seg_tab;
	unsigned long long *tab_first, *sub_last;
	unsigned long long batch_hi;
};

void run_stage_a(const KParams &P, const BatchBufs &B, const uint8_t *seq, const uint8_t *qual, int64_t n_pos, uint64_t *out1, hipStream_t st, hipEvent_t *ev);
void run_stage_a_onepass(const KParams &P, const BatchBufs &B, const uint8_t *seq, const uint8_t *qual, int64_t n_pos, uint64_t *out1, hipStream_t st, hipEvent_t *ev);
void run_stage_b(const KParams &P, const BatchBufs &B, const uint64_t *in1, const uint32_t *seg_beg, const uint32_t *seg_end, int n_seg, int segs_per_bucket,
                 const uint32_t *row_base, const uint32_t *bucket_start, uint64_t n_rec_bound, hipStream_t st, hipEvent_t *ev);
void run_pack_rows(const KParams &P, const BatchBufs &B, int n_ranks, uint32_t row_w, uint32_t *rows, hipStream_t st);
void run_seg_setup_mg(const KParams &P, int rw_dwords, const uint32_t *rows, uint32_t row_w, int n_ranks, int s_lo, int s_hi, uint32_t cap, uint32_t *seg, unsigned long long *total, hipStream_t st);
void run_batch(const KParams &P, const BatchBufs &B, const uint8_t *seq, const uint8_t *qual, int64_t n_pos, hipStream_t st, hipEvent_t *ev);
int bloom_lds_bytes(const KParams &P);
bool bloom3fm_geometry_ok(const KParams &P);
bool bloom3_geometry_ok(const KParams &P);
BFCG_LOCAL bool scatter2_big_ok(const KParams &P);
hipError_t set_bloom_lds_attr(const KParams &P);
void run_query(const KParams &P, const uint8_t *seq, int64_t n_pos, const void *bloom, uint8_t *flags, hipStream_t st);
void run_kcov(const KParams &P, const uint8_t *seq, int64_t n_pos, int min_occ, const void *tab, uint8_t *flags, uint16_t *out, hipStream_t st);
void run_streak(int k, float min_frac, const uint8_t *flags, const uint64_t *off, uint64_t n_reads, int32_t *out_start, int32_t *out_end, hipStream_t st);
void run_hash_only(const KParams &P, const uint8_t *seq, const uint8_t *qual, int64_t n_pos, uint64_t *out, hipStream_t st);
void run_table_replay(const KParams &P, unsigned long long *tab, const uint64_t *src, uint64_t n, unsigned long long *stats, uint64_t *ovf, uint32_t ovf_cap,
                      unsigned long long *first, unsigned long long *sub_last, hipStream_t st);
void run_seg_rehash(const KParams &P, const unsigned long long *old_tab, int old_shift, int old_blk, unsigned long long *new_tab, uint32_t n_fine, hipStream_t st);
void run_seg_replay(const KParams &P, unsigned long long *seg_tab, const uint64_t *src, uint64_t n, unsigned long long *stats, uint64_t *ovf, uint32_t ovf_cap, hipStream_t st);
void run_seg_to_table(const KParams &P, const unsigned long long *seg_tab, uint32_t n_fine, unsigned long long *tab, unsigned long long *stats, uint64_t *ovf, uint32_t ovf_cap, hipStream_t st);
hipError_t set_seg_lds_attr(void);
hipError_t set_scatter1wc_lds_attr(void);
void run_commit_pages(const KParams &P, const BatchBufs &B, uint32_t n_fine, uint32_t pages, hipStream_t st);
#define BFCG_SEG_MAX_SHIFT 14
#define BFCG_SEG_TOTAL_MAX 24
void run_table_rehash(const KParams &P, const unsigned long long *old_tab, int cshift_old, unsigned long long *new_tab,
                      const unsigned long long *old_first, unsigned long long *new_first, hipStream_t st);

BFCG_LOCAL int fail(const char *fmt, ...) __attribute__((format(printf, 1, 2)));
#define BFCG_CK(call) do { hipError_t e_ = (call); if (e_ != hipSuccess) return bfcg::fail("%s failed: %s (%s:%d)", #call, hipGetErrorString(e_), __FILE__, __LINE__); } while (0)
#define BFCG_CKN(cleanup, call) do { hipError_t e_ = (call); if (e_ != hipSuccess) { bfcg::fail("%s failed: %s (%s:%d)", #call, hipGetErrorString(e_), __FILE__, __LINE__); cleanup; (void)hipGetLastError(); return NULL; } } while (0)

struct resident_t { const void *host; void *dev; int device, n_shift, k, l_pre, cshift; };
BFCG_LOCAL int resident_put(const resident_t &r);
BFCG_LOCAL void *resident_take(const void *host, int device, int n_shift, int k, int l_pre, int cshift);

const unsigned long long *ctx_borrow_table(::bfcg_ctx *c, KParams *P, int *device);
int ctx_table_k(::bfcg_ctx *c);
const unsigned long long *kcov_table(::bfcg_kcov *t, KParams *P, int *device);
int kcov_adopted(::bfcg_kcov *t);
BFCG_LOCAL uint64_t lookup_cap();
BFCG_LOCAL int profile_launch(::bfcg_kmers *t, const uint8_t *h_seq, const uint8_t *d_seq, uint64_t n_pos);
template <typename T> int grow(T *&buf, uint64_t &cap, uint64_t need, const char *what)
{
	if (need <= cap) return 0;
	(void)hipFree(buf); buf = NULL; cap = 0;
	hipError_t e = hipMalloc(&buf, need);
	if (e != hipSuccess) { buf = NULL; (void)hipGetLastError(); return fail("no room for %s of %llu bytes: %s", what, (unsigned long long)need, hipGetErrorString(e)); }
	cap = need;
	return 0;
}

}
```

bfc_amd/csrc/bfcg_kernels.hip:

```cpp
#include <hip/hip_runtime.h>
#include <stdint.h>
#include <stdlib.h>
#include <string.h>
#include <stdio.h>
#include "kmer_dev.h"
#include "bfcg_internal.h"
#include "bfcg_dev.h"
#include "bfcg_k1.h"

using namespace bfcg;

#define WAVE 64








template <typename W> __device__ __forceinline__ uint32_t fine_id(const KParams &P, uint64_t y0, uint64_t y1)
{
	W m = kmask<W>(P.k);
	uint64_t hash = bloom_hash<W>(P.k, (W)y0, (W)y1, m);
// ... 436 lines not shown
	const uint32_t n_rows = row_base[n_seg];
	const int64_t row = xcd_tile(blockIdx.x, n_rows);
	if (row >= n_rows) return;
	const int b1 = row_bucket(row_base, n_seg, (uint32_t)row);
	const uint32_t tile = (uint32_t)row - row_base[b1];
	const uint32_t s = seg_beg[b1], e = seg_end[b1];
	const uint32_t imp = (P.f_base >> P.F2) + (uint32_t)(b1 / segs_per_bucket);
	const uint32_t *rowp = ONEPASS2 ? nullptr : rows2 + (size_t)row * nb2;
	for (int i = threadIdx.x; i < nb2; i += BT) cnt[i] = 0;
	__syncthreads();
	RecW<RW> w[S];
	uint32_t br[S];
#pragma unroll
	for (int j = 0; j < S; ++j) {
		uint64_t i = (uint64_t)s + (uint64_t)tile * TILE + j * BT + threadIdx.x;
		br[j] = 0xffffffffu;
		if (i < e) {
			uint64_t y0, y1; uint32_t idx; bool hi;
			w[j] = rec_load<RW>(in + i * RW);
			if (!rec_dead<RW>(w[j])) {
				uint32_t b;
				if constexpr (FAST2) b = (w[j].d[0] >> P.R) & (uint32_t)(nb2 - 1);
				else { Rec<RW>::unpack(w[j], RG, imp, y0, y1, idx, hi); b = fine_id<W>(P, y0, y1) & (nb2 - 1); }
				br[j] = (b << 16) | atomicAdd(&cnt[b], 1u);
			}
		}
	}
	__syncthreads();
	uint32_t n_live;
	{
		const uint32_t tot = block_scan_excl<BT>(cnt, nb2, wsum2);
		n_live = tot;
		__syncthreads();
	}
	constexpr int NQ = (BFCG_MAXB + BT - 1) / BT;
	uint32_t q_base[NQ], q_ex[NQ], q_c[NQ];
	if (!ONEPASS2) {
#pragma unroll
		for (int u = 0; u < NQ; ++u) {
			const int i = threadIdx.x + u * BT;
			q_base[u] = 0; q_ex[u] = 0; q_c[u] = 0;
			if (i < nb2) q_base[u] = rowp[i] - cnt[i];
		}
	}
	if (ONEPASS2) {
		const uint32_t f0 = (uint32_t)(b1 / segs_per_bucket) << P.F2;
#pragma unroll
		for (int u = 0; u < NQ; ++u) {
			const int i = threadIdx.x + u * BT;
			q_base[u] = 0; q_ex[u] = 0; q_c[u] = 0;
			if (i < nb2) {
				q_ex[u] = cnt[i]; q_c[u] = (i + 1 < nb2 ? cnt[i + 1] : n_live) - q_ex[u];
				if (q_c[u]) q_base[u] = atomicAdd(&O2.cnt2[f0 + i], q_c[u]);
			}
		}
	}
#pragma unroll
	for (int j = 0; j < S; ++j) {
		if (br[j] != 0xffffffffu) {
			const uint32_t b = br[j] >> 16, pos = cnt[b] + (br[j] & 0xffffu);
#pragma unroll
			for (int t = 0; t < RW; ++t) stage[(size_t)pos * RW + t] = w[j].d[t];
			if (KEEP_BK) sbk[pos] = (unsigned short)b;
		}
	}
	__syncthreads();
	{
		const uint32_t f0 = (uint32_t)(b1 / segs_per_bucket) << P.F2;
#pragma unroll
		for (int u = 0; u < NQ; ++u) {
			const int i = threadIdx.x + u * BT;
			if (i < nb2) {
				uint32_t base = q_base[u];
				if (ONEPASS2) {
					if (q_c[u] && base + q_c[u] > O2.cap2) { O2.flags[2] = 1; base = 0; }
					base = (f0 + (uint32_t)i) * O2.cap2 + base - q_ex[u];
				}
				gdelta[i] = base;
			}
		}
	}
	__syncthreads();
	const uint32_t n_in = n_live;
	for (uint32_t pos = threadIdx.x; pos < n_in; pos += BT) {
		RecW<RW> rec;
#pragma unroll
		for (int t = 0; t < RW; ++t) rec.d[t] = stage[(size_t)pos * RW + t];
		uint32_t b;
		if (KEEP_BK) b = sbk[pos];
		else if constexpr (FAST2) b = (rec.d[0] >> P.R) & (uint32_t)(nb2 - 1);
		else { uint64_t y0, y1; uint32_t idx; bool hi; Rec<RW>::unpack(rec, RG, imp, y0, y1, idx, hi); b = fine_id<W>(P, y0, y1) & (uint32_t)(nb2 - 1); }
		const uint64_t dst = (uint32_t)(pos + gdelta[b]);
		rec_store<RW>(out + dst * RW, rec);
	}
}

__global__ __launch_bounds__(1024) void k_seg_setup(KParams P, const uint32_t *__restrict__ cursor, uint32_t cap, const uint32_t *flags, int tile2,
                                                    uint32_t *__restrict__ seg_beg, uint32_t *__restrict__ seg_end, uint32_t *__restrict__ row_base,
                                                    uint32_t *__restrict__ bucket_start)
{
	__shared__ uint32_t s_rows[1024], s_recs[1024];
	__shared__ uint32_t s_poison;
	const int nb1 = 1 << P.F1, t = threadIdx.x;
	if (t == 0) s_poison = flags[0];
	__syncthreads();
	const bool poison = s_poison != 0;
	uint32_t len[8], rows = 0, recs = 0;
#pragma unroll
	for (int x = 0; x < 8; ++x) {
		uint32_t l = 0;
		if (t < nb1 && !poison) { l = cursor[((size_t)x * nb1 + t) * 32]; if (l > cap) l = cap; }
		len[x] = l; rows += (l + tile2 - 1) / tile2; recs += l;
	}
	s_rows[t] = rows; s_recs[t] = recs;
	__syncthreads();
	for (int o = 1; o < 1024; o <<= 1) {
		const uint32_t a = t >= o ? s_rows[t - o] : 0, b = t >= o ? s_recs[t - o] : 0;
		__syncthreads();
		s_rows[t] += a; s_recs[t] += b;
		__syncthreads();
	}
	if (t < nb1) {
		uint32_t r = s_rows[t] - rows;
		bucket_start[t] = s_recs[t] - recs;
#pragma unroll
		for (int x = 0; x < 8; ++x) {
			const uint32_t seg = (uint32_t)t * 8u + x, beg = seg * cap;
			seg_beg[seg] = beg; seg_end[seg] = beg + len[x]; row_base[seg] = r;
			r += (len[x] + tile2 - 1) / tile2;
		}
	}
	if (t == nb1 - 1) { row_base[(size_t)nb1 * 8] = s_rows[t]; bucket_start[nb1] = s_recs[t]; }
}

__global__ __launch_bounds__(256) void k_pack_rows(const uint32_t *__restrict__ seg_end, const uint32_t *__restrict__ flags, int nb_loc, uint32_t cap, uint32_t row_w,
                                                  uint32_t *__restrict__ rows)
{
	const uint32_t p = blockIdx.x, n = (uint32_t)nb_loc * 8u;
	const uint32_t poison = flags[0];
	for (uint32_t i = threadIdx.x; i < n; i += blockDim.x) {
		const uint32_t seg = p * n + i;
		rows[(size_t)p * row_w + i] = poison ? 0u : seg_end[seg] - seg * cap;
	}
	if (threadIdx.x == 0) { rows[(size_t)p * row_w + n] = poison; rows[(size_t)p * row_w + n + 1] = 0u; }
}
__global__ __launch_bounds__(1024) void k_seg_setup_mg(const uint32_t *__restrict__ rows, uint32_t row_w, int N, int s_lo, int s_hi, int nb_loc, uint32_t cap, int tile2,
                                                       uint32_t *__restrict__ seg_beg, uint32_t *__restrict__ seg_end, uint32_t *__restrict__ row_base,
                                                       uint32_t *__restrict__ bucket_start, unsigned long long *__restrict__ total)
{
	__shared__ uint32_t s_rows[1024], s_recs[1024];
	__shared__ uint32_t s_poison;
	const int t = threadIdx.x, nt = nb_loc * N, k = t / N, s = t - k * N;
	if (t == 0) s_poison = 0;
	__syncthreads();
	if (t < N && rows[(size_t)t * row_w + (size_t)nb_loc * 8] != 0) s_poison = 1;
	__syncthreads();
	const bool poison = s_poison != 0;
	uint32_t len[8], nrow = 0, recs = 0;
#pragma unroll
	for (int x = 0; x < 8; ++x) {
		uint32_t l = 0;
		if (t < nt && !poison && s >= s_lo && s < s_hi) { l = rows[(size_t)s * row_w + (size_t)k * 8 + x]; if (l > cap) l = cap; }
		len[x] = l; nrow += (l + tile2 - 1) / tile2; recs += l;
	}
	s_rows[t] = nrow; s_recs[t] = recs;
	__syncthreads();
	for (int o = 1; o < 1024; o <<= 1) {
		const uint32_t a = t >= o ? s_rows[t - o] : 0, b = t >= o ? s_recs[t - o] : 0;
		__syncthreads();
		s_rows[t] += a; s_recs[t] += b;
		__syncthreads();
	}
	if (t < nt) {
		uint32_t r = s_rows[t] - nrow;
		if (s == 0) bucket_start[k] = s_recs[t] - recs;
// ... 1239 lines not shown
{
	const int a = P.k - P.rec_n;
	return P.k >= P.bf_shift - 9 && a >= 1 && a <= 31 && a + P.k >= 32 && (P.rec_n == 0 || P.rec_lo + P.rec_n <= 31) && !getenv("BFCG_NO_FAST_K1");
}

template <typename W, int RW>
static void run_stage_a_t(const KParams &P, const BatchBufs &B, const uint8_t *seq, const uint8_t *qual, int64_t n_pos, uint32_t *out1, hipStream_t st, hipEvent_t *ev)
{
	constexpr int T1 = bfcg_tile1_of_rw(RW), T2 = bfcg_tile_of_rw(RW);
	const int nb1 = 1 << P.F1;
	const int64_t tiles1 = (n_pos + T1 - 1) / T1;
	const int n_chunks = (int)((tiles1 + SCAN_CH - 1) / SCAN_CH);
	if (ev) hipEventRecord(ev[0], st);
	const unsigned g1 = (unsigned)(((tiles1 + 7) / 8) * 8);
	hipLaunchKernelGGL((k_hist1<W, T1, BT1>), dim3(g1), dim3(BT1), 0, st, P, seq, qual, n_pos, B.rows1, B.stats);
	hipLaunchKernelGGL(k_colsum, dim3(n_chunks), dim3(256), 0, st, B.rows1, (int)tiles1, nb1, B.chunk1);
	hipLaunchKernelGGL(k_scan_top, dim3(1), dim3(nb1 < 64 ? 64 : nb1), 0, st, B.chunk1, n_chunks, nb1, B.start1, B.row_base, T2);
	hipLaunchKernelGGL(k_apply, dim3(n_chunks), dim3(256), 0, st, B.rows1, (int)tiles1, nb1, B.chunk1);
	if (ev) hipEventRecord(ev[1], st);
	hipLaunchKernelGGL(have(scatter1_kernel<W, RW>(S1V_TWO_PASS), "k_scatter1", S1V_TWO_PASS, RW), dim3(g1), dim3(BTS1), scatter1_lds_bytes(RW, nb1, false, P.rec_n), st, P, seq, qual, n_pos, B.rows1, out1, OnePass{nullptr, 0u, nullptr, nullptr, 0u, 0u, 0u, 0u});
	if (ev) hipEventRecord(ev[2], st);
}

template <typename W, int RW>
static void run_stage_a_onepass_t(const KParams &P, const BatchBufs &B, const uint8_t *seq, const uint8_t *qual, int64_t n_pos, uint32_t *out1, hipStream_t st, hipEvent_t *ev)
{
	constexpr int T1 = bfcg_tile1_of_rw(RW), T2 = bfcg_tile_of_rw(RW);
	const int nb1 = 1 << P.F1;
	const int64_t tiles1 = (n_pos + T1 - 1) / T1;
	if (ev) hipEventRecord(ev[0], st);
	hipMemsetAsync(B.op_cursor, 0, ((size_t)8 * nb1 * 32 + 32) * sizeof(uint32_t), st);
	hipMemsetAsync(B.op_flags, 0, 4 * sizeof(uint32_t), st);
	if (ev) hipEventRecord(ev[1], st);
	unsigned g1 = (unsigned)(((tiles1 + 7) / 8) * 8);
	const size_t lds1 = scatter1_lds_bytes(RW, nb1, true, P.rec_n);
	OnePass OP{B.op_cursor, B.op_cap, B.op_flags, B.stats, 1u, B.op_own_lo, B.op_own_n, B.op_own_delta};
	{
		static int n_cu = 0;
		if (!n_cu) { hipDeviceProp_t pr; int dev = 0; n_cu = (hipGetDevice(&dev) == hipSuccess && hipGetDeviceProperties(&pr, dev) == hipSuccess) ? pr.multiProcessorCount : 256; }
		int per_cu = (int)((size_t)160 * 1024 / (lds1 + 4400)); if (per_cu > 2) per_cu = 2; if (per_cu < 1) per_cu = 1;
		const char *e = getenv("BFCG_S1_WGS"); if (e && atoi(e) > 0) per_cu = atoi(e);
		const unsigned gp = (unsigned)(n_cu * per_cu) & ~7u;
		if (gp >= 8 && gp < g1) g1 = gp;
	}
	if (B.cnt_live) {
		const char *e = getenv("BFCG_S1_CHUNK");
		const int forced = e ? atoi(e) : 0;
		uint32_t ch = 32;
		while (ch > 1 && (uint64_t)(g1 / 8) * (ch / 2) * 36 > B.op_cap) ch >>= 1;
		OP.chunk = forced > 0 ? (uint32_t)forced : ch;
	}
	WcPlan wc;
	const bool fast = RW == 3 && scatter1_fast(P);
	const int v = !fast ? S1V_ONEPASS : sizeof(W) == 8 && P.k == 33 ? S1V_FAST_K33 : S1V_FAST;
	if ((fast || RW == 4) && B.cnt_live && scatter1_wc_plan(P, OP, RW, n_pos, &wc)) run_scatter1_wc(P, seq, qual, n_pos, out1, OP, wc, st);
	else hipLaunchKernelGGL(have(scatter1_kernel<W, RW>(v), "k_scatter1", v, RW), dim3(g1), dim3(BTS1), lds1, st, P, seq, qual, n_pos, nullptr, out1, OP);
	dbg_sync(st, "k_scatter1 (one pass)");
	uint32_t *sg = B.op_seg;
	hipLaunchKernelGGL(k_seg_setup, dim3(1), dim3(1024), 0, st, P, B.op_cursor, B.op_cap, B.op_flags, (RW == 3 && P.l2_big) ? TILE2_BIG : T2, sg, sg + 8 * nb1, sg + 16 * nb1, sg + 24 * nb1 + 1);
	dbg_sync(st, "k_seg_setup");
	if (ev) hipEventRecord(ev[2], st);
}

static inline bool scatter2_fast(const KParams &P)
{
	const int a = P.k - P.rec_n;
	return P.k >= P.bf_shift - 9 && P.F2 > 0 && P.R + P.F2 <= 31 && a >= P.R + P.F2 && P.rec_lo == P.R + P.F2 && !getenv("BFCG_NO_FAST_S2");
}

static inline bool bloom_fast3(const KParams &P)
{
	const int a = P.k - P.rec_n, up = P.rec_n ? P.rec_lo : P.bf_shift - 9, sh_x = P.k - (P.bf_shift - 9), sh_y1 = P.k - P.F;
	return P.k >= P.bf_shift - 9 && P.bf_shift + 9 <= 2 * P.k && a >= 1 && a <= 31 && a + P.k >= 32 && (P.rec_n == 0 || P.rec_lo + P.rec_n <= 31)
	       && up <= a && sh_x >= 0 && sh_x <= 31 && sh_y1 >= 0 && sh_y1 <= 32 && (P.rec_n == 0 || P.rec_lo + P.rec_n == P.bf_shift - 9) && P.R <= up && !getenv("BFCG_NO_FAST_BLOOM");
}

bool bloom3fm_geometry_ok(const KParams &P)
{
	const int up = P.rec_n ? P.rec_lo : P.bf_shift - 9, a = P.k - P.rec_n, io = a + P.k + 1;
	return bfcg_rec_dwords(P.k, P.rec_n) == 4 && P.n_hashes == 4 && P.R <= 8 && P.k >= P.bf_shift + 9 && (P.rec_n == 0 || P.rec_lo + P.rec_n == P.bf_shift - 9)
	       && P.R <= up && up >= 1 && up <= 31 && a >= up + 18 && io + 32 <= 128;
}
bool bloom3_geometry_ok(const KParams &P) { return bfcg_rec_dwords(P.k, P.rec_n) == 3 && P.n_hashes == 4 && P.R <= 8 && bloom_fast3(P); }
bool scatter2_big_ok(const KParams &P) { return bfcg_rec_dwords(P.k, P.rec_n) == 3 && scatter2_fast(P); }

static dim3 seg_grid(const KParams &P, uint32_t n_fine, uint32_t bt)
{
	const uint32_t ub = (uint32_t)(P.seg_shift - P.seg_blk);
	const uint64_t wgs = (uint64_t)n_fine << ub;
	static const bool force2d = getenv("BFCG_SEG_GRID2D") != nullptr;
	if (wgs * bt < (1ULL << 32) && !force2d) return dim3((unsigned)wgs, 1u);
	return dim3(n_fine, 1u << ub);
}
static void launch_commit_seg(const KParams &P, const BloomArgs &A, int nfine, hipStream_t st)
{
	const BloomK k = commit_seg_kernel(P.seg_blk);
	hipLaunchKernelGGL(k.fn, seg_grid(P, (uint32_t)nfine, (uint32_t)k.bt), dim3(k.bt), commit_seg_lds_bytes(P.seg_blk), st, P, A);
	dbg_sync(st, "k_commit_seg");
}
void run_commit_pages(const KParams &P, const BatchBufs &B, uint32_t n_fine, uint32_t pages, hipStream_t st)
{
	BloomArgs A;
	memset(&A, 0, sizeof(A));
	A.stats = B.stats; A.tab_ovf = B.tab_ovf; A.tab_ovf_cap = B.tab_ovf_cap; A.ovf_cnt = B.stats + (size_t)ST_SLOTS * ST_N; A.seg_tab = B.seg_tab; A.n_fine = n_fine;
	A.ho = B.ho; A.ho_stride = B.ho_stride; A.ho_cur = B.ho_cur; A.ho_mark = B.ho_mark; A.ho_mark_stride = B.ho_mark_stride; A.ho_pages = pages; A.ho_keys = B.ho_keys;
	launch_commit_seg(P, A, (int)n_fine, st);
}

template <typename W, int RW>
static std::pair<const uint32_t *, const uint32_t *> run_level2_t(const KParams &P, const BatchBufs &B, const uint32_t *in1, const uint32_t *seg_beg, const uint32_t *seg_end, int n_seg,
                                                                  int segs_per_bucket, const uint32_t *row_base, const uint32_t *bucket_start, uint64_t n_rec_bound, hipStream_t st)
{
	if (P.F2 == 0) return {in1, bucket_start};
	const int nb_loc = n_seg / segs_per_bucket, nfine = nb_loc << P.F2;
	int v = S2V_TWO_PASS;
	if (B.cap2) {
		const bool fast = (RW == 3 || RW == 4) && scatter2_fast(P);
		v = !fast ? S2V_ONEPASS : RW == 3 && P.l2_big ? S2V_FAST_BIG : S2V_FAST;
		hipMemsetAsync(B.cnt2, 0, sizeof(uint32_t) * (size_t)nfine, st);
	} else {
		hipLaunchKernelGGL((k_hist2<W, RW, bfcg_tile_of_rw(RW), BT2>), dim3(level2_grid(n_rec_bound, bfcg_tile_of_rw(RW), n_seg)), dim3(BT2), 0, st, P, in1, seg_beg, seg_end, n_seg, segs_per_bucket, row_base, B.rows2);
		hipLaunchKernelGGL(k_scan2, dim3(nb_loc), dim3((1 << P.F2) < 64 ? 64 : (1 << P.F2)), 0, st, P, bucket_start, segs_per_bucket, row_base, B.rows2, B.start2, B.cnt_live);
	}
	const Scatter2K k = scatter2_kernel<W, RW>(v);
	hipLaunchKernelGGL(have(k.fn, "k_scatter2", v, RW), dim3(level2_grid(n_rec_bound, k.tile, n_seg)), dim3(k.bt), scatter2_lds_bytes(RW, k.tile, 1 << P.F2), st, P, in1, seg_beg, seg_end, n_seg, segs_per_bucket, row_base,
	                   B.cap2 ? nullptr : B.rows2, (uint32_t *)B.recs2, B.cap2 ? OnePass2{B.cnt2, B.cap2, B.op_flags} : OnePass2{nullptr, 0u, nullptr});
	dbg_sync(st, "level 2");
	return {(const uint32_t *)B.recs2, B.start2};
}

template <typename W, int RW>
static BloomArgs run_bloom_t(const KParams &P, const BatchBufs &B, const uint32_t *fine_recs, const uint32_t *fine_start, int nfine, hipStream_t st)
{
	BloomArgs A;
	memset(&A, 0, sizeof(A));
	A.recs = fine_recs; A.start = fine_start; A.bloom = B.bloom; A.bloom_hi = B.bloom_hi; A.table = B.table; A.stats = B.stats;
	A.tab_ovf = B.tab_ovf; A.tab_ovf_cap = B.tab_ovf_cap; A.ovf_cnt = B.stats + (size_t)ST_SLOTS * ST_N; A.pool = B.pool; A.pool_slices = B.pool_slices; A.seen_out = B.seen_out;
	A.agg_out = B.agg_out; A.agg_cnt = B.agg_cnt; A.n_fine = (uint32_t)nfine; A.stream_out = nullptr; A.seg_tab = nullptr;
	A.ord.first = B.tab_first; A.ord.sub_last = B.sub_last; A.batch_hi = B.batch_hi;
	A.cnt2 = nullptr; A.cap2 = 0; A.flags = B.op_flags; A.sticky = B.op_sticky;
	if (P.F2 > 0 && B.cap2) { A.cnt2 = B.cnt2; A.cap2 = B.cap2; }
	else if (P.F2 > 0 && B.cnt_live) A.cnt2 = B.cnt_live;
	const bool h4 = P.n_hashes == 4;
	if (P.filter_mode && B.bloom_hi) {
		if (RW == 4 && P.b3fm) run_bloom3fm(P, A, nfine, (size_t)bloom_lds_bytes(P), st);
		else launch_bloom<W, RW>(!h4 ? BV_FM_ANYH : P.bloom_bt == 1024 ? BV_FM_1024 : BV_FM, P, A, nfine, st);
	} else if (P.seg && B.seg_tab && (B.stream_out || B.ho)) {
		A.stream_out = B.stream_out; A.seg_tab = B.seg_tab; A.table = nullptr; A.agg_out = nullptr;
		A.ho = B.ho; A.ho_stride = B.ho_stride; A.ho_cur = B.ho_cur; A.ho_mark = B.ho_stride ? B.ho_mark + (size_t)B.ho_page * B.ho_mark_stride : nullptr;
		if (RW == 3 && P.b3 && (P.b3_cold || !P.dedupe)) run_bloom3(P, A, nfine, (size_t)bloom_lds_bytes(P), st);
		else launch_bloom<W, RW>(!h4 ? BV_SEG_ANYH : RW == 3 && bloom_fast3(P) ? BV_SEG_F3 : BV_SEG, P, A, nfine, st);
	} else if (B.stream && B.stream_out && !P.track && h4) {
		A.stream_out = B.stream_out;
		launch_bloom<W, RW>(BV_STREAM, P, A, nfine, st);
	} else if (P.track) launch_bloom<W, RW>(h4 ? BV_TRACK : BV_TRACK_ANYH, P, A, nfine, st);
	else launch_bloom<W, RW>(!h4 ? BV_ANYH : P.bloom_bt == 1024 ? BV_1024 : BV_512, P, A, nfine, st);
	return A;
}

template <typename W, int RW>
static void run_commit_t(const KParams &P, const BatchBufs &B, BloomArgs &A, int nfine, hipStream_t st)
{
	const auto waves = [&] { return dim3((unsigned)((nfine + 4 * COMMIT_RPW - 1) / (4 * COMMIT_RPW))); };
	if (A.seg_tab) {
		if (B.ho_stride == 0 || B.ho_commit) {
			A.ho_mark = B.ho_mark; A.ho_mark_stride = B.ho_mark_stride; A.ho_pages = B.ho_page + 1; A.ho_keys = B.ho_keys;
			launch_commit_seg(P, A, nfine, st);
		}
	} else if (A.stream_out) hipLaunchKernelGGL((k_commit_stream<W, RW>), waves(), dim3(256), 0, st, P, A);
	else if (B.agg_out && nfine > (1 << 18)) hipLaunchKernelGGL((P.track ? k_commit<W, true, true> : k_commit<W, false, true>), waves(), dim3(256), 0, st, P, A);
	else if (B.agg_out) hipLaunchKernelGGL((P.track ? k_commit<W, true, false> : k_commit<W, false, false>), dim3((unsigned)(((uint64_t)nfine * P.ag_cap + 255) / 256)), dim3(256), 0, st, P, A);
}

template <typename W, int RW>
static void run_stage_b_t(const KParams &P, const BatchBufs &B, const uint32_t *in1, const uint32_t *seg_beg, const uint32_t *seg_end, int n_seg,
                          int segs_per_bucket, const uint32_t *row_base, const uint32_t *bucket_start, uint64_t n_rec_bound, hipStream_t st, hipEvent_t *ev)
{
	const int nfine = (n_seg / segs_per_bucket) << P.F2;
	const auto [fine_recs, fine_start] = run_level2_t<W, RW>(P, B, in1, seg_beg, seg_end, n_seg, segs_per_bucket, row_base, bucket_start, n_rec_bound, st);
	if (ev) hipEventRecord(ev[3], st);
	BloomArgs A = run_bloom_t<W, RW>(P, B, fine_recs, fine_start, nfine, st);
	if (ev) hipEventRecord(ev[4], st);
	if (A.seg_tab || A.stream_out) dbg_sync(st, "k_bloom");
	run_commit_t<W, RW>(P, B, A, nfine, st);
	if (A.flags) hipLaunchKernelGGL(k_seal, dim3(1), dim3(1), 0, st, B.op_flags, B.op_sticky);
	if (ev) hipEventRecord(ev[5], st);
}

#define DISPATCH_W(fn, ...) do { const int rw_ = bfcg_rec_dwords(P.k, P.rec_n); \
	if (P.k <= 32) { if (rw_ == 3) fn<uint32_t, 3>(__VA_ARGS__); else fn<uint32_t, 4>(__VA_ARGS__); } \
	else if (rw_ == 3) fn<uint64_t, 3>(__VA_ARGS__); else if (rw_ == 4) fn<uint64_t, 4>(__VA_ARGS__); else fn<uint64_t, 5>(__VA_ARGS__); } while (0)

void run_stage_a(const KParams &P, const BatchBufs &B, const uint8_t *seq, const uint8_t *qual, int64_t n_pos, uint64_t *out1, hipStream_t st, hipEvent_t *ev)
{ DISPATCH_W(run_stage_a_t, P, B, seq, qual, n_pos, (uint32_t *)out1, st, ev); }

void run_stage_a_onepass(const KParams &P, const BatchBufs &B, const uint8_t *seq, const uint8_t *qual, int64_t n_pos, uint64_t *out1, hipStream_t st, hipEvent_t *ev)
{ DISPATCH_W(run_stage_a_onepass_t, P, B, seq, qual, n_pos, (uint32_t *)out1, st, ev); }

void run_pack_rows(const KParams &P, const BatchBufs &B, int n_ranks, uint32_t row_w, uint32_t *rows, hipStream_t st)
{
	const int nb1 = 1 << P.F1;
	hipLaunchKernelGGL(k_pack_rows, dim3((unsigned)n_ranks), dim3(256), 0, st, B.op_seg + (size_t)8 * nb1, B.op_flags, nb1 / n_ranks, B.op_cap, row_w, rows);
}
void run_seg_setup_mg(const KParams &P, int rw_dwords, const uint32_t *rows, uint32_t row_w, int n_ranks, int s_lo, int s_hi, uint32_t cap, uint32_t *seg, unsigned long long *total, hipStream_t st)
{
	const int nb1 = 1 << P.F1, nb_loc = nb1 / n_ranks, n_seg = nb1 * 8;
	hipLaunchKernelGGL(k_seg_setup_mg, dim3(1), dim3(1024), 0, st, rows, row_w, n_ranks, s_lo, s_hi, nb_loc, cap, bfcg_tile_of_rw(rw_dwords), seg, seg + n_seg, seg + 2 * n_seg, seg + 3 * n_seg + 1, total);
}

void run_stage_b(const KParams &P, const BatchBufs &B, const uint64_t *in1, const uint32_t *seg_beg, const uint32_t *seg_end, int n_seg, int segs_per_bucket,
                 const uint32_t *row_base, const uint32_t *bucket_start, uint64_t n_rec_bound, hipStream_t st, hipEvent_t *ev)
{ DISPATCH_W(run_stage_b_t, P, B, (const uint32_t *)in1, seg_beg, seg_end, n_seg, segs_per_bucket, row_base, bucket_start, n_rec_bound, st, ev); }

void run_batch(const KParams &P, const BatchBufs &B, const uint8_t *seq, const uint8_t *qual, int64_t n_pos, hipStream_t st, hipEvent_t *ev)
{
	run_stage_a(P, B, seq, qual, n_pos, B.recs1, st, ev);
	run_stage_b(P, B, B.recs1, B.start1, B.start1 + 1, 1 << P.F1, 1, B.row_base, B.start1, (uint64_t)n_pos, st, ev);
}

int bloom_lds_bytes(const KParams &P)
{
	const size_t second = P.filter_mode ? ((size_t)64 << P.R) : P.seg ? 0 : (size_t)P.ag_cap * ((P.k > 32 ? 24 : 16) + (P.track ? 8 : 0));
	if (P.b3fm) return (int)(((size_t)128 << P.R) + ((size_t)2 << P.R) * 4 + 16 + (size_t)P.list_cap * 10 + 16);
	if (P.b3 && P.b3_cold) return (int)(((size_t)64 << P.R) + ((size_t)2 << P.R) * 4 + 16 + (size_t)P.list_cap * 12 + 16);
	return (int)(((size_t)64 << P.R) + (size_t)P.fs_cap * 4 + second + (size_t)P.list_cap * (P.b3 ? 10 : 8) + 16);
}

template <typename W, int RW> static void register_lds_t(int lds, hipError_t *err)
{
	hipError_t e = hipSuccess;
	for (int v = 0; v < S1V_N && e == hipSuccess; ++v) if (const Scatter1Fn fn = scatter1_kernel<W, RW>(v)) e = set_max_lds((const void *)fn, scatter1_lds_bytes(RW, BFCG_MAXB, v != S1V_TWO_PASS, 1));
	for (int v = 0; v < S2V_N && e == hipSuccess; ++v) if (const Scatter2K k = scatter2_kernel<W, RW>(v); k.fn) e = set_max_lds((const void *)k.fn, scatter2_lds_bytes(RW, k.tile, BFCG_MAXB));
	for (int v = 0; v < BV_N && e == hipSuccess; ++v) if (const BloomK k = bloom_kernel<W, RW>(v); k.fn) e = set_max_lds((const void *)k.fn, (size_t)lds);
	for (int blk = 11; blk <= 13 && e == hipSuccess; ++blk)
		e = set_max_lds((const void *)commit_seg_kernel(blk).fn, commit_seg_lds_bytes(BFCG_SEG_MAX_SHIFT));
	if (RW == 3 && e == hipSuccess) e = set_bloom3_lds_attr(lds);
	if (RW == 4 && e == hipSuccess) e = set_bloom3fm_lds_attr(lds);
	*err = e;
}
hipError_t set_bloom_lds_attr(const KParams &P)
{ hipError_t e = hipSuccess; DISPATCH_W(register_lds_t, bloom_lds_bytes(P), &e); return e; }

void run_query(const KParams &P, const uint8_t *seq, int64_t n_pos, const void *bloom, uint8_t *flags, hipStream_t st)
{
	const int64_t tiles = (n_pos + TILE1 - 1) / TILE1;
	const unsigned g = (unsigned)(((tiles + 7) / 8) * 8);
	const char *eq = getenv("BFCG_QUERY4");
	const int q4 = eq ? atoi(eq) : -1;
	if (P.n_hashes == 4 && P.bf_shift <= 41 && (q4 == 1 || (q4 != 0 && P.bf_shift >= 35))) {
		if (P.k <= 32) hipLaunchKernelGGL((k_query4<uint32_t, TILE1, BT1>), dim3(g), dim3(BT1), 0, st, P, seq, n_pos, (const unsigned int *)bloom, reinterpret_cast<unsigned long long *>(flags));
		else hipLaunchKernelGGL((k_query4<uint64_t, TILE1, BT1>), dim3(g), dim3(BT1), 0, st, P, seq, n_pos, (const unsigned int *)bloom, reinterpret_cast<unsigned long long *>(flags));
		return;
	}
	const bool coop = P.bf_shift >= 35;
	if (P.k <= 32) {
		if (coop) hipLaunchKernelGGL((k_query<uint32_t, TILE1, BT1, true>), dim3(g), dim3(BT1), 0, st, P, seq, n_pos, (const unsigned int *)bloom, reinterpret_cast<unsigned long long *>(flags));
		else hipLaunchKernelGGL((k_query<uint32_t, TILE1, BT1, false>), dim3(g), dim3(BT1), 0, st, P, seq, n_pos, (const unsigned int *)bloom, reinterpret_cast<unsigned long long *>(flags));
	} else {
		if (coop) hipLaunchKernelGGL((k_query<uint64_t, TILE1, BT1, true>), dim3(g), dim3(BT1), 0, st, P, seq, n_pos, (const unsigned int *)bloom, reinterpret_cast<unsigned long long *>(flags));
		else hipLaunchKernelGGL((k_query<uint64_t, TILE1, BT1, false>), dim3(g), dim3(BT1), 0, st, P, seq, n_pos, (const unsigned int *)bloom, reinterpret_cast<unsigned long long *>(flags));
	}
// ... 53 lines not shown
```

bfc_amd/csrc/bfcg_kmers.hip:

```cpp
#include <hip/hip_runtime.h>
#include <stdint.h>
#include <stdio.h>
#include <stdlib.h>
#include <string.h>
#include "bfc_gpu.h"
#include "bfcg_internal.h"
#include "bfc_host.h"
#include "bfcg_kdec.h"

namespace {

enum { BT = 256, WAVES = BT / 64, HIST_BINS = 256 + 64, HIST_COPIES = 8 , HIST_UNROLL = 4 };
enum { LIST_STEPS = 8, LIST_WAVE = LIST_STEPS * 128 , LIST_BLK = WAVES * LIST_WAVE  };
enum { SCAN_BT = 1024, SCAN_PER = 8 };

__device__ __forceinline__ int lane_id() { return (int)(threadIdx.x & 63); }

__global__ __launch_bounds__(BT) void k_tab_hist(const ulonglong2 *__restrict__ tab, uint64_t n_pairs, uint64_t span_pairs, int cshift,
                                                 unsigned long long *__restrict__ hist, uint32_t *__restrict__ sizes)
{
	__shared__ uint32_t h[WAVES * HIST_COPIES][HIST_BINS];
	for (int i = threadIdx.x; i < WAVES * HIST_COPIES * HIST_BINS; i += BT) (&h[0][0])[i] = 0;
	__syncthreads();
	const int lane = lane_id(), wave = threadIdx.x >> 6;
	uint32_t *mine = h[wave * HIST_COPIES + (lane & (HIST_COPIES - 1))];
	const uint64_t gw = (uint64_t)blockIdx.x * WAVES + wave;
	const uint64_t p_lo = gw * span_pairs, p_hi = p_lo + span_pairs < n_pairs ? p_lo + span_pairs : n_pairs;
	const int g = cshift >= 7 ? 64 : cshift >= 1 ? 1 << (cshift - 1) : 1;
	const uint64_t gmask = g == 64 ? ~0ULL : ((1ULL << g) - 1) << (lane & ~(g - 1));
	uint64_t run_sub = ~0ULL; uint32_t run_cnt = 0;
	for (uint64_t p = p_lo; p < p_hi; p += 64 * HIST_UNROLL) {
		ulonglong2 v[HIST_UNROLL];
#pragma unroll
		for (int j = 0; j < HIST_UNROLL; ++j) {
			const uint64_t q = p + (uint64_t)j * 64 + lane;
			v[j] = q < p_hi ? tab[q] : make_ulonglong2(0, 0);
		}
#pragma unroll
		for (int j = 0; j < HIST_UNROLL; ++j) {
			const uint64_t q = p + (uint64_t)j * 64 + lane;
			const uint64_t x = v[j].x, y = v[j].y;
			if (x) { atomicAdd(&mine[x & 0xff], 1u); atomicAdd(&mine[256 + (x >> 8 & 0x3f)], 1u); }
			if (y) { atomicAdd(&mine[y & 0xff], 1u); atomicAdd(&mine[256 + (y >> 8 & 0x3f)], 1u); }
			const uint64_t bx = __ballot(x != 0), by = __ballot(y != 0);
			if (cshift == 0) {
				if (x) sizes[2 * q] = 1;
				if (y) sizes[2 * q + 1] = 1;
			} else if (g < 64) {
				const uint32_t n = __popcll(bx & gmask) + __popcll(by & gmask);
				if ((lane & (g - 1)) == 0 && n && q < p_hi) atomicAdd(&sizes[(2 * q) >> cshift], n);
			} else {
				const uint64_t sub = (2 * (p + (uint64_t)j * 64)) >> cshift;
				if (sub != run_sub) {
					if (lane == 0 && run_cnt) atomicAdd(&sizes[run_sub], run_cnt);
					run_sub = sub; run_cnt = 0;
				}
				run_cnt += __popcll(bx) + __popcll(by);
			}
		}
	}
	if (g == 64 && lane == 0 && run_cnt) atomicAdd(&sizes[run_sub], run_cnt);
	__syncthreads();
	for (int b = threadIdx.x; b < HIST_BINS; b += BT) {
		unsigned long long s = 0;
		for (int c = 0; c < WAVES * HIST_COPIES; ++c) s += h[c][b];
		if (s) atomicAdd(&hist[b], s);
	}
}

struct ListGeom { uint64_t s_lo, s_hi, base; int k, l_pre, cshift, min_cnt, min_diff; };

__device__ __forceinline__ void list_load(const ulonglong2 *__restrict__ tab, const ListGeom &G, uint64_t wave_first, ulonglong2 v[LIST_STEPS])
{
	const int lane = lane_id();
#pragma unroll
	for (int j = 0; j < LIST_STEPS; ++j) {
		const uint64_t s = wave_first + (uint64_t)j * 128 + 2 * lane;
		ulonglong2 w = make_ulonglong2(0, 0);
		if (s < G.s_hi) w = tab[s >> 1];
		if (s < G.s_lo || !kdec::keep(w.x, G.min_cnt, G.min_diff)) w.x = 0;
		if (s + 1 < G.s_lo || s + 1 >= G.s_hi || !kdec::keep(w.y, G.min_cnt, G.min_diff)) w.y = 0;
		v[j] = w;
	}
}

__global__ __launch_bounds__(BT) void k_list_count(const ulonglong2 *__restrict__ tab, ListGeom G, uint32_t *__restrict__ blk_cnt)
{
	__shared__ uint32_t wsum[WAVES];
	const int wave = threadIdx.x >> 6;
	ulonglong2 v[LIST_STEPS];
	list_load(tab, G, G.base + (uint64_t)blockIdx.x * LIST_BLK + (uint64_t)wave * LIST_WAVE, v);
// ... 173 lines not shown
	if (!cnt) return -1;
	memcpy(cnt, h, 256 * 8); memcpy(high, h + 256, 64 * 8);
	uint64_t max = 0; int mode = -1;
	for (int i = 3; i < 256; ++i) if (cnt[i] > max) { max = cnt[i]; mode = i; }
	return mode;
}

extern "C" int bfcg_kmers_hist(bfcg_kmers_t *t, uint64_t cnt[256], uint64_t high[64])
{
	if (!cnt || !high) { bfcg::fail("bad arguments to bfcg_kmers_hist"); return -2; }
	return bfcg_kmers_hist_sizes(t, cnt, high, NULL);
}

extern "C" int bfcg_kmers_sub_sizes(bfcg_kmers_t *t, uint32_t *sizes)
{
	if (!sizes) return bfcg::fail("bad arguments to bfcg_kmers_sub_sizes");
	return bfcg_kmers_hist_sizes(t, NULL, NULL, sizes) == -2 ? -1 : 0;
}

extern "C" int bfcg_kmers_list(bfcg_kmers_t *t, int min_cnt, int min_diff, uint32_t sub_lo, uint32_t sub_hi, uint64_t *y, uint16_t *cnt_high, uint64_t cap, uint64_t *n)
{
	if (!t || !n) return bfcg::fail("bad arguments to bfcg_kmers_list");
	if (!kdec::decodable(t->k)) return bfcg::fail("k-mers cannot be listed for k=%d: the table's key is lossless only for k <= %d (sizes and histogram work for any k)", t->k, (int)kdec::MAX_K);
	if (sub_lo > sub_hi || (uint64_t)sub_hi > 1ULL << t->l_pre) return bfcg::fail("sub-table range [%u, %u) outside [0, 2^%d]", sub_lo, sub_hi, t->l_pre);
	if (cap && (!y || !cnt_high)) return bfcg::fail("bfcg_kmers_list needs output buffers for cap=%llu", (unsigned long long)cap);
	*n = 0; t->last_ms = 0;
	if (sub_lo == sub_hi) return 0;
	BFCG_CK(hipSetDevice(t->device));
	ListGeom G;
	G.s_lo = (uint64_t)sub_lo << t->cshift; G.s_hi = (uint64_t)sub_hi << t->cshift; G.base = G.s_lo & ~1ULL;
	G.k = t->k; G.l_pre = t->l_pre; G.cshift = t->cshift; G.min_cnt = min_cnt; G.min_diff = min_diff;
	const uint64_t n_blk = (G.s_hi - G.base + LIST_BLK - 1) / LIST_BLK, per = SCAN_BT * SCAN_PER, n_pad = (n_blk + per - 1) / per * per;
	if (n_blk >= 1ULL << 24) return bfcg::fail("sub-table range of %llu slots is too large for one listing: walk it in pieces", (unsigned long long)(G.s_hi - G.s_lo));
	if (n_pad > t->blk_cap) {
		(void)hipFree(t->d_cnt); (void)hipFree(t->d_off); t->d_cnt = NULL; t->d_off = NULL; t->blk_cap = 0;
		BFCG_CK(hipMalloc(&t->d_cnt, n_pad * 4)); BFCG_CK(hipMalloc(&t->d_off, (n_pad + 1) * 8));
		t->blk_cap = n_pad;
	}
	float ms1 = 0, ms2 = 0;
	if (n_pad > n_blk) BFCG_CK(hipMemsetAsync(t->d_cnt + n_blk, 0, (n_pad - n_blk) * 4, t->st));
	BFCG_CK(hipEventRecord(t->e0, t->st));
	hipLaunchKernelGGL(k_list_count, dim3((unsigned)n_blk), dim3(BT), 0, t->st, (const ulonglong2 *)t->table, G, t->d_cnt);
	hipLaunchKernelGGL(k_list_scan, dim3(1), dim3(SCAN_BT), 0, t->st, t->d_cnt, n_pad, t->d_off);
	BFCG_CK(hipEventRecord(t->e1, t->st));
	BFCG_CK(hipGetLastError());
	unsigned long long total = 0;
	BFCG_CK(hipMemcpyAsync(&total, t->d_off + n_pad, 8, hipMemcpyDeviceToHost, t->st));
	BFCG_CK(hipStreamSynchronize(t->st));
	BFCG_CK(hipEventElapsedTime(&ms1, t->e0, t->e1));
	t->last_ms = ms1;
	*n = total;
	if (total > cap) return 1;
	if (total == 0) return 0;
	if (total > t->out_cap) {
		(void)hipFree(t->d_y); (void)hipFree(t->d_ch); t->d_y = NULL; t->d_ch = NULL; t->out_cap = 0;
		BFCG_CK(hipMalloc(&t->d_y, total * 16)); BFCG_CK(hipMalloc(&t->d_ch, total * 2));
		t->out_cap = total;
	}
	BFCG_CK(hipEventRecord(t->e0, t->st));
	hipLaunchKernelGGL(k_list_emit, dim3((unsigned)n_blk), dim3(BT), 0, t->st, (const ulonglong2 *)t->table, G, t->d_off, t->d_y, t->d_ch, (uint64_t)total);
	BFCG_CK(hipEventRecord(t->e1, t->st));
	BFCG_CK(hipGetLastError());
	BFCG_CK(hipMemcpyAsync(y, t->d_y, total * 16, hipMemcpyDeviceToHost, t->st));
	BFCG_CK(hipMemcpyAsync(cnt_high, t->d_ch, total * 2, hipMemcpyDeviceToHost, t->st));
	BFCG_CK(hipStreamSynchronize(t->st));
	BFCG_CK(hipEventElapsedTime(&ms2, t->e0, t->e1));
	t->last_ms = ms1 + ms2;
	return 0;
}

extern "C" float bfcg_kmers_last_ms(bfcg_kmers_t *t) { return t ? t->last_ms : 0.0f; }


extern "C" int bfcg_kmer_decode_host(int k, int l_pre, uint32_t sub, uint64_t slot, uint64_t y[2])
{
	if (!kdec::decodable(k) || l_pre < 0 || l_pre > BFC_CH_MAXPRE || (k <= 32 ? 2 * k - l_pre < 0 || 2 * k - l_pre > BFC_CH_KEYBITS : k - l_pre < 0)) return -1;
	kdec::decode(k, l_pre, sub, slot, y[0], y[1]);
	uint64_t Y0, Y1, Z0, Z1;
	kdec::slot_to_hash(k, l_pre, sub, slot, Y0, Y1);
	kdec::kmer_to_hash(k, y[0], y[1], Z0, Z1);
	return Y0 == Z0 && Y1 == Z1 ? 0 : -1;
}

extern "C" void bfcg_kmer_2str(int k, const uint64_t y[2], char *buf)
{
	for (int l = 0; l < k; ++l) buf[k - 1 - l] = "ACGT"[(y[1] >> l & 1) << 1 | (y[0] >> l & 1)];
	buf[k] = 0;
}

static inline char *put_u32(char *p, uint32_t v)
{
	char tmp[10]; int n = 0;
	do { tmp[n++] = (char)('0' + v % 10); v /= 10; } while (v);
	while (n) *p++ = tmp[--n];
	return p;
}

extern "C" uint64_t bfcg_kmers_format(int k, const uint64_t *y, const uint16_t *cnt_high, uint64_t n, char *buf)
{
	char *p = buf;
	for (uint64_t i = 0; i < n; ++i) {
		const uint64_t a = y[2 * i], b = y[2 * i + 1];
		for (int l = 0; l < k; ++l) p[k - 1 - l] = "ACGT"[(b >> l & 1) << 1 | (a >> l & 1)];
		p += k; *p++ = '\t';
		p = put_u32(p, cnt_high[i] & 0xff); *p++ = '\t';
		p = put_u32(p, cnt_high[i] >> 8 & 0x3f); *p++ = '\n';
	}
	return (uint64_t)(p - buf);
}

extern "C" uint64_t bfcg_kmers_format_sizes(const uint32_t *sizes, uint64_t n, char *buf)
{
	char *p = buf;
	for (uint64_t i = 0; i < n; ++i) { p = put_u32(p, sizes[i]); *p++ = '\n'; }
	return (uint64_t)(p - buf);
}
```

bfc_amd/csrc/kmer_dev.h:

```cpp
#pragma once
#include <hip/hip_runtime.h>
#include <stdint.h>

namespace bfcg {

template <typename W> __device__ __forceinline__ W kmask(int k)
{
	return k >= (int)(8 * sizeof(W)) ? ~W(0) : (W(1) << k) - 1;
}

template <typename W> __device__ __forceinline__ W mix_k(W v, W m)
{
	v = (~v + (v << 21)) & m;
	v ^= v >> 24;
	v = (v + (v << 3) + (v << 8)) & m;
	v ^= v >> 14;
	v = (v + (v << 2) + (v << 4)) & m;
	v ^= v >> 28;
	v = (v + (v << 31)) & m;
	return v;
}

__device__ __forceinline__ uint32_t brev_w(uint32_t v) { return __brev(v); }
__device__ __forceinline__ uint64_t brev_w(uint64_t v) { return __brevll(v); }
// ... 38 lines not shown
	v.hi = ((uint32_t)(d >> 32) + v.hi * 0x1FFFFFu) & mh; v.lo = (uint32_t)d;
	v.lo ^= __builtin_amdgcn_alignbit(v.hi, v.lo, 24); if (!KC || kh > 24) v.hi ^= v.hi >> 24;
	d = (uint64_t)v.lo * 265u;
	v.hi = ((uint32_t)(d >> 32) + v.hi * 265u) & mh; v.lo = (uint32_t)d;
	v.lo ^= __builtin_amdgcn_alignbit(v.hi, v.lo, 14); if (!KC || kh > 14) v.hi ^= v.hi >> 14;
	d = (uint64_t)v.lo * 21u;
	v.hi = ((uint32_t)(d >> 32) + v.hi * 21u) & mh; v.lo = (uint32_t)d;
	v.lo ^= __builtin_amdgcn_alignbit(v.hi, v.lo, 28); if (!KC || kh > 28) v.hi ^= v.hi >> 28;
	d = (uint64_t)v.lo * 0x80000001u;
	v.hi = ((uint32_t)(d >> 32) + v.hi) & mh; v.lo = (uint32_t)d;
	return v;
}

template <int KC> __device__ __forceinline__ void kmer_hash_from_windows2(int k_, uint32_t wl_lo, uint32_t wl_hi, uint32_t wh_lo, uint32_t wh_hi, U2 &y0, U2 &y1)
{
	const int k = KC ? KC : k_, kh = k - 32, s = 32 - kh, t = k >> 1;
	const uint32_t mh = (1u << kh) - 1u;
	const uint32_t sel = 0u - ((wh_lo >> t) & (wh_lo >> (k - 1 - t)) & 1u);
	const uint32_t rl = __brev(wl_lo), rh = __brev(wh_lo);
	U2 a, b;
	a.lo = (__builtin_amdgcn_alignbit(rl, __brev(wl_hi), s) & ~sel) | (~wl_lo & sel);
	a.hi = ((rl >> s) & ~sel) | (~wl_hi & sel);
	b.lo = (__builtin_amdgcn_alignbit(rh, __brev(wh_hi), s) & ~sel) | (~wh_lo & sel);
	b.hi = ((rh >> s) & ~sel) | (~wh_hi & sel);
	const U2 h0 = mix2<KC>(u2_split(u2_join(a) + u2_join(b)), k);
	U2 x; x.lo = h0.lo ^ b.lo; x.hi = h0.hi ^ b.hi;
	const U2 h1 = mix2<KC>(x, k);
	y0 = u2_split(u2_join(h0) + u2_join(h1)); y0.hi &= mh;
	y1 = h1;
}

template <typename W> __device__ __forceinline__ uint64_t bloom_hash(int k, W y0, W y1, W m)
{
	W h0 = (y0 - y1) & m;
	return ((uint64_t)(h0 ^ y1) << k) | (uint64_t)y0;
}

__device__ __forceinline__ uint32_t ch_subkey(int k, int l_pre, uint64_t y0, uint64_t y1, uint64_t &key)
{
	if (k <= 32) {
		int t = 2 * k - l_pre;
		uint64_t z = (y0 << k) | y1;
		key = ((z & ((1ULL << t) - 1)) << 14) | 1;
		return (uint32_t)(z >> t);
	} else {
		int t = k - l_pre;
		int sh = (t + k < 50) ? k : 50 - t;
		key = ((((y0 & ((1ULL << t) - 1)) << sh) ^ y1) << 14) | 1;
		return (uint32_t)(y0 >> t);
	}
}

__device__ __forceinline__ int ch_get_dev(int k, int l_pre, int cshift, const unsigned long long *__restrict__ tab, uint64_t y0, uint64_t y1)
{
	uint64_t key;
	const uint32_t sub = ch_subkey(k, l_pre, y0, y1, key);
	const uint32_t cmask = (1u << cshift) - 1;
	const unsigned long long *reg = tab + ((uint64_t)sub << cshift);
	uint32_t pos = (uint32_t)(key >> 14) & cmask;
	for (uint32_t probe = 0; probe <= cmask; ++probe, pos = (pos + 1) & cmask) {
		const unsigned long long cur = reg[pos];
		if (cur == 0) return -1;
		if ((cur >> 14) == (key >> 14)) return (int)(cur & 0x3fff);
	}
	return -1;
}

struct SegGeom { int k, lo, hi; };
__host__ __device__ __forceinline__ uint64_t seg_id(const SegGeom g, uint64_t y0, uint64_t y1)
{
	const uint64_t low = y0 & ((1ULL << g.lo) - 1), up = g.hi < g.k ? y0 >> g.hi : 0;
	return low | up << g.lo | y1 << (g.k - (g.hi - g.lo));
}
__host__ __device__ __forceinline__ void seg_unpack(const SegGeom g, uint64_t f_global, uint64_t id, uint64_t &y0, uint64_t &y1)
{
	const int nimp = g.hi - g.lo, kb = g.k - nimp;
	const uint64_t imp = f_global & ((1ULL << nimp) - 1);
	const uint64_t kept = id & ((1ULL << kb) - 1);
	y0 = (kept & ((1ULL << g.lo) - 1)) | imp << g.lo | (g.hi < g.k ? (kept >> g.lo) << g.hi : 0);
	y1 = id >> kb;
}
__host__ __device__ __forceinline__ uint32_t seg_home(uint64_t id) { return (uint32_t)((id * 0x9E3779B97F4A7C15ULL) >> 38); }

struct BloomAddr {
	uint64_t blk;
	uint32_t h1, h2;
};
__device__ __forceinline__ BloomAddr bloom_addr(uint64_t hash, int bf_shift)
{
	BloomAddr a;
	int x = bf_shift - 9;
	a.blk = hash & ((1ULL << x) - 1);
	a.h1 = (uint32_t)(hash >> x) & 511u;
	a.h2 = (uint32_t)(hash >> bf_shift) & 511u;
	if ((a.h2 & 31u) == 0) a.h2 = (a.h2 + 1) & 511u;
	return a;
}
__device__ __forceinline__ uint32_t bloom_next(uint32_t &z, uint32_t h2)
{
	while (z < 8) z = (z + h2) & 511u;
	uint32_t r = z;
	z = (z + h2) & 511u;
	return r;
}

}
```

include/bfc_gpu.h:

```cpp
#ifndef BFC_GPU_H
#define BFC_GPU_H

#include <stdint.h>

#ifdef __cplusplus
extern "C" {
#endif


typedef struct { uint64_t x[4]; } bfc_kmer_t;

#define BFC_BLK_SHIFT 9
#define BFC_BLK_MASK  ((1 << BFC_BLK_SHIFT) - 1)
typedef struct { int n_shift, n_hashes; uint8_t *b; } bfc_bf_t;

bfc_bf_t *bfc_bf_init(int n_shift, int n_hashes);
void      bfc_bf_destroy(bfc_bf_t *b);
int       bfc_bf_insert(bfc_bf_t *b, uint64_t hash);
int       bfc_bf_get(const bfc_bf_t *b, uint64_t hash);

#define BFC_CH_KEYBITS 50
#define BFC_CH_MAXPRE  24
struct bfc_ch_s;
typedef struct bfc_ch_s bfc_ch_t;
// ... 86 lines not shown
bfc_ch_t *bfcg_group_export_table(bfcg_group_t *g);
bfc_bf_t *bfcg_group_export_bloom(bfcg_group_t *g, int which);
bfc_bf_t *bfcg_group_export_bloom_resident(bfcg_group_t *g, int which);

void *bfcg_dev_alloc(bfcg_ctx_t *c, uint64_t bytes);
void  bfcg_dev_free(bfcg_ctx_t *c, void *p);
int   bfcg_h2d(bfcg_ctx_t *c, void *dst, const void *src, uint64_t bytes);
int   bfcg_d2h(bfcg_ctx_t *c, void *dst, const void *src, uint64_t bytes);
void *bfcg_host_alloc(uint64_t bytes);
void  bfcg_host_free(void *p);

int bfcg_stats(bfcg_ctx_t *c, uint64_t out[BFCG_ST_N]);
int bfcg_progress(bfcg_ctx_t *c, uint64_t *calls, uint64_t *final, uint64_t *keys_of, int n);
int bfcg_table_info(bfcg_ctx_t *c, int out[4]);
int bfcg_partition_info(bfcg_ctx_t *c, uint64_t out[2]);
uint64_t bfcg_s1wc_launches(void);
uint64_t bfcg_stream_batches(bfcg_ctx_t *c);

int bfcg_last_batch_ms(bfcg_ctx_t *c, float out[6]);
int bfcg_stage_ms(bfcg_ctx_t *c, double out[6], uint64_t *n_batches, int reset);

int bfcg_bloom_to_host(bfcg_ctx_t *c, int which , uint8_t *dst);
bfc_bf_t *bfcg_export_bloom(bfcg_ctx_t *c, int which);
bfc_bf_t *bfcg_export_bloom_resident(bfcg_ctx_t *c, int which);
void bfcg_resident_drop(const void *bf);
bfc_ch_t *bfcg_export_table(bfcg_ctx_t *c);
bfc_ch_t *bfcg_export_table_resident(bfcg_ctx_t *c);

int bfc_ingest_digest(const char *fn, uint64_t chunk_size, uint64_t cap, int n_threads, uint64_t out[7]);
int bfc_ingest_planes_digest(const char *fn, uint64_t chunk_size, uint64_t cap, int n_threads, int q, int direct, uint64_t out[7]);
int bfc_pgz_digest(const char *fn, int n_threads, uint64_t chunk, uint64_t window, uint64_t out[5]);

bfc_ch_t *bfc_ch_union(const bfc_ch_t *const *tabs, int n);

int      bfc_ch_get_lpre(const bfc_ch_t *ch);
uint64_t bfc_ch_export_sorted(const bfc_ch_t *ch, uint32_t *sizes, uint64_t *slots);

typedef struct bfcg_trim bfcg_trim_t;
bfcg_trim_t *bfcg_trim_create(int k, const bfc_bf_t *bf, int device, uint64_t max_pos, uint64_t max_reads);
void bfcg_trim_destroy(bfcg_trim_t *t);
int bfcg_trim_batch(bfcg_trim_t *t, const uint8_t *h_seq, const uint8_t *d_seq, uint64_t n_pos, const uint64_t *h_off, uint64_t n_reads,
                    float min_frac, int32_t *start, int32_t *end);
float bfcg_trim_last_ms(bfcg_trim_t *t);
int bfcg_trim_adopted(bfcg_trim_t *t);
void *bfcg_trim_dev_seq(bfcg_trim_t *t);

typedef struct bfcg_kcov bfcg_kcov_t;
bfcg_kcov_t *bfcg_kcov_create(const bfc_ch_t *ch, int device, uint64_t max_pos);
bfcg_kcov_t *bfcg_kcov_attach(bfcg_ctx_t *ctx, uint64_t max_pos);
void bfcg_kcov_destroy(bfcg_kcov_t *t);
int bfcg_kcov_batch(bfcg_kcov_t *t, const uint8_t *h_seq, const uint8_t *d_seq, uint64_t n_pos, int min_occ, uint16_t *out);
float bfcg_kcov_last_ms(bfcg_kcov_t *t);
void *bfcg_kcov_dev_seq(bfcg_kcov_t *t);
void *bfcg_kcov_dev_out(bfcg_kcov_t *t);

typedef struct bfcg_ec bfcg_ec_t;
bfcg_ec_t *bfcg_ec_create(const bfc_ch_t *ch, const bfc_opt_t *opt, int device, uint64_t max_pos, uint64_t max_reads);
bfcg_ec_t *bfcg_ec_attach(bfcg_ctx_t *ctx, const bfc_opt_t *opt, uint64_t max_pos, uint64_t max_reads);
int   bfcg_ec_batch(bfcg_ec_t *e, uint8_t *seq, uint8_t *qual, uint64_t n_pos, const uint64_t *off, uint64_t n_reads, uint32_t *aux, uint32_t *aux2);
void  bfcg_ec_destroy(bfcg_ec_t *e);
float bfcg_ec_last_ms(bfcg_ec_t *e);
uint64_t bfcg_ec_host_reads(bfcg_ec_t *e);
uint64_t bfcg_ec_last_lookups(bfcg_ec_t *e);
uint64_t bfcg_ec_retry_reads(bfcg_ec_t *e);
int   bfcg_ec_adopted(bfcg_ec_t *e);
int   bfcg_ec1_host(const bfc_ch_t *ch, const bfc_opt_t *opt, int mode, char *seq, char *qual, uint32_t *aux, uint32_t *aux2);
int   bfcg_ec_batch_refine(bfcg_ec_t *e, uint8_t *seq, uint8_t *qual, uint64_t n_pos, const uint64_t *off, uint64_t n_reads,
                           const uint32_t *ori_aux, const uint32_t *ori_aux2, uint32_t *aux, uint32_t *aux2);
int   bfcg_ec1_host_refine(const bfc_ch_t *ch, const bfc_opt_t *opt, int mode, char *seq, char *qual, uint32_t ori_aux, uint32_t ori_aux2,
                           uint32_t *aux, uint32_t *aux2);
int   bfcg_ec_parse_stats(const char *comment, uint32_t *aux, uint32_t *aux2);

typedef struct bfcg_kmers bfcg_kmers_t;
bfcg_kmers_t *bfcg_kmers_create(const bfc_ch_t *ch, int device);
bfcg_kmers_t *bfcg_kmers_attach(bfcg_ctx_t *ctx);
void  bfcg_kmers_destroy(bfcg_kmers_t *t);
int   bfcg_kmers_info(bfcg_kmers_t *t, int out[3]);
int   bfcg_kmers_hist(bfcg_kmers_t *t, uint64_t cnt[256], uint64_t high[64]);
int   bfcg_kmers_sub_sizes(bfcg_kmers_t *t, uint32_t *sizes);
int   bfcg_kmers_hist_sizes(bfcg_kmers_t *t, uint64_t cnt[256], uint64_t high[64], uint32_t *sizes);
int   bfcg_kmers_list(bfcg_kmers_t *t, int min_cnt, int min_diff, uint32_t sub_lo, uint32_t sub_hi, uint64_t *y, uint16_t *cnt_high, uint64_t cap, uint64_t *n);
float bfcg_kmers_last_ms(bfcg_kmers_t *t);
int   bfcg_kmer_decode_host(int k, int l_pre, uint32_t sub, uint64_t slot, uint64_t y[2]);
void  bfcg_kmer_2str(int k, const uint64_t y[2], char *buf);
uint64_t bfcg_kmers_format(int k, const uint64_t *y, const uint16_t *cnt_high, uint64_t n, char *buf);
uint64_t bfcg_kmers_format_sizes(const uint32_t *sizes, uint64_t n, char *buf);
int   bfcg_kmers_lookup(bfcg_kmers_t *t, const uint64_t *y, uint64_t n, int16_t *out, uint64_t *n_found);
int   bfcg_kmers_profile(bfcg_kmers_t *t, const uint8_t *h_seq, const uint8_t *d_seq, uint64_t n_pos, int16_t *out);
int   bfcg_kmer_from_str(int k, const char *s, uint64_t y[2]);
int   bfcg_kmer_occ_host(const bfc_ch_t *ch, const uint64_t y[2]);
void  bfcg_kmers_occ_host(const bfc_ch_t *ch, const uint64_t *y, uint64_t n, int16_t *out);
uint64_t bfcg_kmers_parse(int k, const char *text, uint64_t len, uint64_t *y, uint64_t cap, uint64_t *bad_line);
uint64_t bfcg_lookup_format(const char *text, uint64_t len, const int16_t *occ, uint64_t n, char *buf);
uint64_t bfcg_profile_format(const int16_t *occ, uint64_t n, char *buf);
int   bfcg_kmers_read_stats(bfcg_kmers_t *t, const uint8_t *h_seq, const uint8_t *d_seq, uint64_t n_pos, const uint64_t *h_off, uint64_t n_reads,
                            int min_cov, int32_t *out);
int   bfcg_read_stats_host(const bfc_ch_t *ch, const uint8_t *seq, uint64_t n_pos, const uint64_t *off, uint64_t n_reads, int min_cov, int32_t *out);
uint64_t bfcg_read_stats_format(const int32_t *out, uint64_t n_reads, char *buf);

int bfcg_hash_positions(bfcg_ctx_t *c, const uint8_t *h_seq, const uint8_t *h_qual, uint64_t n_pos, uint64_t *out);
int bfcg_seen_flags(bfcg_ctx_t *c, uint8_t *dst, uint64_t n_pos);

#ifdef __cplusplus
}
#endif
#endif
```

Before: 40660.

## Pre-pack level-2 records into bloom3 entry layout with embedded hash bits

The level-2 scatter now rewrites each 3-dword record into the final table-entry encoding, and stores the extra hash bits the bloom address needs in the high bits. The bloom3 kernel can then build the address with a few shifts and take the entry by masking, instead of decoding the record twice. This moves per-record decode work out of the bloom kernel, which revisits records, and into the scatter pass. In exchange the scatter does more ALU work, there are more kernel template variants, and the layout is only valid when the geometry checks pass. An env var can turn it off.

```diff
diff --git a/bfc_amd/_lib.py b/bfc_amd/_lib.py
--- a/bfc_amd/_lib.py
+++ b/bfc_amd/_lib.py
@@ -147,6 +147,10 @@
     "bfcg_kmers_last_ms": (C.c_float, [C.c_void_p]),
     "bfcg_kmer_decode_host": (C.c_int, [C.c_int, C.c_int, C.c_uint32, C.c_uint64, u64p]),
     "bfcg_kmer_2str": (None, [C.c_int, u64p, C.c_char_p]),
+    "bfcg_rec2_b3_pack_host": (C.c_int, [C.c_void_p, C.c_uint64, C.c_void_p, C.c_void_p, C.c_void_p]),
+    "bfcg_rec2_addr_host": (C.c_int, [C.c_void_p, C.c_int, C.c_uint64, C.c_void_p, C.c_void_p, C.c_void_p]),
+    "bfcg_rec2_entry_host": (C.c_int, [C.c_void_p, C.c_int, C.c_uint64, C.c_void_p, C.c_void_p]),
+    "bfcg_rec2_entry_unpack_host": (C.c_int, [C.c_void_p, C.c_uint64, C.c_void_p, C.c_void_p, C.c_void_p, C.c_void_p]),
     "bfcg_kmers_format": (C.c_uint64, [C.c_int, C.c_void_p, C.c_void_p, C.c_uint64, C.c_void_p]),
     "bfcg_kmers_format_sizes": (C.c_uint64, [C.c_void_p, C.c_uint64, C.c_void_p]),
     "bfcg_kmers_lookup": (C.c_int, [C.c_void_p, C.c_void_p, C.c_uint64, C.c_void_p, u64p]),
diff --git a/bfc_amd/api.py b/bfc_amd/api.py
--- a/bfc_amd/api.py
+++ b/bfc_amd/api.py
@@ -323,10 +323,13 @@
         self.L.bfcg_table_info(self.ctx, out)
         return dict(segments=bool(out[0]), seg_shift=out[1], tab_cshift=out[2], seg_growths=out[3])
 
-    def partition_info(self):
+    def partition_info(self, layout=False):
         out = (C.c_uint64 * 2)()
         self.L.bfcg_partition_info(self.ctx, out)
-        return dict(one_pass=bool(out[0] & 1), level2_one_pass=bool(out[0] & 2), replayed_batches=int(out[1]))
+        d = dict(one_pass=bool(out[0] & 1), level2_one_pass=bool(out[0] & 2), replayed_batches=int(out[1]))
+        if layout:
+            d["rec2_b3"] = bool(out[0] & 4)
+        return d
 
     def s1wc_launches(self):
         return int(self.L.bfcg_s1wc_launches())
diff --git a/bfc_amd/csrc/bfcg_bloom3.hip b/bfc_amd/csrc/bfcg_bloom3.hip
--- a/bfc_amd/csrc/bfcg_bloom3.hip
+++ b/bfc_amd/csrc/bfcg_bloom3.hip
@@ -10,7 +10,7 @@
 #define B3_UND 0x40000000u
 #define B3_SEEN 0x40000000u
 #define B3_COLD_NR 8
-template <int BT, int PF, bool COLD>
+template <int BT, int PF, bool COLD, bool B3>
 __global__ __launch_bounds__(BT, PF <= 2 ? 8 : 6) void k_bloom3(KParams P, BloomArgs A)
 {
 	extern __shared__ __attribute__((aligned(16))) unsigned char smem[];
@@ -49,27 +49,16 @@
 	const uint32_t imp = (P.f_base + f) >> P.F2;
 	const Dec3 D = dec3_geom(P);
 	const int tid = threadIdx.x, lane = tid & 63;
-	const uint32_t mask_a = (1u << D.a) - 1u, imp_sh = D.n ? imp << D.lo : 0u, sh_up = D.lo + D.n;
 #ifdef BFCG_MEASURE
 	const bool timing = BFCG_ABL(P, 64) && tid == 0;
 	long long tq[7] = {0, 0, 0, 0, 0, 0, 0};
 	if (timing) tq[0] = clock64();
 #endif
-	auto addr3 = [&](uint32_t d0, uint32_t d1) -> uint32_t {
-		const uint32_t y0d = d0 & mask_a, upper = y0d >> D.up;
-		const uint32_t y0lo = D.n ? (y0d & D.lowmask) | imp_sh | (upper << sh_up) : y0d;
-		const uint32_t y1lo = __builtin_amdgcn_alignbit(d1, d0, D.a) & D.mk32;
-		const uint32_t hh = upper | (((y0lo - y1lo) ^ y1lo) << D.sh_x);
-		uint32_t h2 = (hh >> 9) & 511u;
-		h2 |= (uint32_t)((h2 & 31u) == 0);
-		return (y0d & D.rmask) | ((hh & 511u) << 8) | (h2 << 17);
-	};
-	auto entry3 = [&](uint32_t d0, uint32_t d1) -> unsigned long long {
-		const unsigned long long AA = d0 | ((unsigned long long)d1 << 32);
-		const unsigned long long y1 = (AA >> D.a) & ((1ULL << P.k) - 1);
-		const uint32_t y0d = d0 & mask_a;
-		const unsigned long long id = (unsigned long long)((y0d & D.rmask) | ((y0d >> D.up) << D.R)) | (y1 << D.sh_y1);
-		return (id << 1) | (unsigned long long)((d1 >> D.sh_flag) & 1u);
+	auto addr3 = [&](uint32_t d0, uint32_t d1) -> uint32_t { if constexpr (B3) return rec3_b3_addr(D, d0, d1); else return rec3_addr(D, imp, d0, d1); };
+	auto entry3 = [&](uint32_t d0, uint32_t d1) -> unsigned long long { if constexpr (B3) return rec3_b3_entry(D, d0, d1); else return rec3_entry(D, d0, d1); };
+	auto entry_at = [&](uint32_t i) -> unsigned long long {
+		if constexpr (B3) { const uint32_t *p = recs + (uint64_t)i * 3; return rec3_b3_entry(D, p[0], p[1]); }
+		else { const RecW<3> r = rec_load<3>(recs + (uint64_t)i * 3); return rec3_entry(D, r.d[0], r.d[1]); }
 	};
 	RecW<3> cur[PF], nxt[PF];
 #pragma unroll
@@ -220,8 +209,7 @@
 					if (lane == 0) o = atomicAdd(&s_emit_n, (uint32_t)__popcll(vote));
 					o = __builtin_amdgcn_readfirstlane(o);
 					if (seen) {
-						const RecW<3> r = rec_load<3>(recs + (uint64_t)lc[li] * 3);
-						ho_base[o + (uint32_t)__builtin_amdgcn_mbcnt_hi((uint32_t)(vote >> 32), __builtin_amdgcn_mbcnt_lo((uint32_t)vote, 0u))] = entry3(r.d[0], r.d[1]);
+						ho_base[o + (uint32_t)__builtin_amdgcn_mbcnt_hi((uint32_t)(vote >> 32), __builtin_amdgcn_mbcnt_lo((uint32_t)vote, 0u))] = entry_at(lc[li]);
 					}
 				}
 			}
@@ -331,10 +319,7 @@
 					uint32_t o = 0;
 					if (lane == 0) o = atomicAdd(&s_emit_n, (uint32_t)__popcll(vote));
 					o = __builtin_amdgcn_readfirstlane(o);
-					if (seen) {
-						const RecW<3> r = rec_load<3>(recs + (uint64_t)lc[li] * 3);
-						ho_base[o + (uint32_t)__popcll(vote & ((1ULL << lane) - 1))] = entry3(r.d[0], r.d[1]);
-					}
+					if (seen) ho_base[o + (uint32_t)__popcll(vote & ((1ULL << lane) - 1))] = entry_at(lc[li]);
 				}
 			}
 			for (uint32_t i = tid; i < (1u << P.R); i += BT) region[i * 16u] &= ~0xffu;
@@ -436,16 +421,20 @@
 namespace bfcg {
 
 typedef void (*BloomFn)(KParams, BloomArgs);
-static BloomFn bloom3_kernel(bool pf2, bool cold)
+static BloomFn bloom3_kernel(bool pf2, bool cold, bool b3)
 {
-	if (cold) return pf2 ? k_bloom3<512, 2, true> : k_bloom3<512, 4, true>;
-	return pf2 ? k_bloom3<512, 2, false> : k_bloom3<512, 4, false>;
+	if (b3) {
+		if (cold) return pf2 ? k_bloom3<512, 2, true, true> : k_bloom3<512, 4, true, true>;
+		return pf2 ? k_bloom3<512, 2, false, true> : k_bloom3<512, 4, false, true>;
+	}
+	if (cold) return pf2 ? k_bloom3<512, 2, true, false> : k_bloom3<512, 4, true, false>;
+	return pf2 ? k_bloom3<512, 2, false, false> : k_bloom3<512, 4, false, false>;
 }
 static hipError_t set_bloom3_max_lds(BloomFn fn, int lds) { return hipFuncSetAttribute((const void *)fn, hipFuncAttributeMaxDynamicSharedMemorySize, lds < BLOOM3_LDS_FLOOR ? BLOOM3_LDS_FLOOR : lds); }
 hipError_t set_bloom3_lds_attr(int lds)
 {
 	hipError_t e = hipSuccess;
-	for (int i = 0; i < 4 && e == hipSuccess; ++i) e = set_bloom3_max_lds(bloom3_kernel(i & 1, i & 2), lds);
+	for (int i = 0; i < 8 && e == hipSuccess; ++i) e = set_bloom3_max_lds(bloom3_kernel(i & 1, i & 2, i & 4), lds);
 	return e;
 }
 
@@ -454,7 +443,7 @@
 	static int pf = 0;
 	if (!pf) { const char *e = getenv("BFCG_B3_PF"); pf = e && atoi(e) == 2 ? 2 : e && atoi(e) == 4 ? 4 : 1; }
 	const bool pf2 = P.b3_cold ? P.b3_warm != 0 : pf == 2 || (pf == 1 && P.b3_warm);
-	hipLaunchKernelGGL(bloom3_kernel(pf2, P.b3_cold != 0), dim3(nfine), dim3(512), lds, st, P, A);
+	hipLaunchKernelGGL(bloom3_kernel(pf2, P.b3_cold != 0, P.rec2_b3 != 0), dim3(nfine), dim3(512), lds, st, P, A);
 }
 
 }
diff --git a/bfc_amd/csrc/bfcg_ctx.hip b/bfc_amd/csrc/bfcg_ctx.hip
--- a/bfc_amd/csrc/bfcg_ctx.hip
+++ b/bfc_amd/csrc/bfcg_ctx.hip
@@ -84,6 +84,7 @@
 	int mg_op2_ok, mg_op2, mg_op2_allowed; uint32_t *mg_seg[4];
 	int mg_slab_ok; int mg_seg_slab[4];
 	uint64_t n_replayed;
+	int rec2_b3;
 	int reused;
 	int seg_no_grow;
 	int seg_cap_shift;
@@ -774,7 +775,7 @@
 	return table_maintain(c);
 }
 
-extern "C" int bfcg_partition_info(bfcg_ctx_t *c, uint64_t out[2]) { out[0] = (uint64_t)((c->onepass ? 1 : 0) | ((c->onepass || (c->mg_op2 && c->mg_op2_allowed)) && c->cap2 ? 2 : 0)); out[1] = c->n_replayed; return 0; }
+extern "C" int bfcg_partition_info(bfcg_ctx_t *c, uint64_t out[2]) { out[0] = (uint64_t)((c->onepass ? 1 : 0) | ((c->onepass || (c->mg_op2 && c->mg_op2_allowed)) && c->cap2 ? 2 : 0) | (c->rec2_b3 ? 4 : 0)); out[1] = c->n_replayed; return 0; }
 extern "C" void bfcg_mg_allow_onepass(bfcg_ctx_t *c, int on) { c->mg_op2_allowed = on != 0; }
 
 extern "C" int bfcg_table_info(bfcg_ctx_t *c, int out[4])
@@ -834,6 +835,7 @@
 static int enqueue_stage_b(bfcg_ctx_t *c, int b, BatchBufs &Bt, const KParams &Pt, const StageB &w)
 {
 	if (handover_begin(c, Bt, b, w.slabs, w.call) != 0) return -1;
+	c->rec2_b3 = stage_b_rec2_b3(Pt, Bt);
 	run_stage_b(Pt, Bt, w.in1, w.seg_beg, w.seg_end, w.n_seg, w.segs_per_bucket, w.row_base, w.bucket_start, w.rec_bound, c->st, c->evt[b]);
 	if (handover_end(c, Bt, b) != 0) return -1;
 	if (w.queued) {
diff --git a/bfc_amd/csrc/bfcg_dev.h b/bfc_amd/csrc/bfcg_dev.h
--- a/bfc_amd/csrc/bfcg_dev.h
+++ b/bfc_amd/csrc/bfcg_dev.h
@@ -96,17 +96,7 @@
 __device__ __forceinline__ bool batch_poisoned(const BloomArgs &A) { return (A.sticky && *A.sticky) || (A.flags && (A.flags[0] | A.flags[2])); }
 
 
-struct Dec3 { int ok, a, lo, n, up, sh_x, R, sh_flag, sh_y1; uint32_t lowmask, rmask, mk32; };
-__device__ __forceinline__ Dec3 dec3_geom(const KParams &P)
-{
-	Dec3 g;
-	g.a = P.k - P.rec_n; g.lo = P.rec_lo; g.n = P.rec_n; g.up = P.rec_n ? P.rec_lo : P.bf_shift - 9; g.sh_x = P.k - (P.bf_shift - 9);
-	g.R = P.R; g.sh_flag = g.a + P.k - 32; g.sh_y1 = P.k - P.F;
-	g.lowmask = P.rec_n ? (1u << (P.rec_lo & 31)) - 1u : 0xffffffffu; g.rmask = (1u << P.R) - 1u; g.mk32 = P.k >= 32 ? 0xffffffffu : (1u << P.k) - 1u;
-	g.ok = P.k >= P.bf_shift - 9 && P.bf_shift + 9 <= 2 * P.k && g.a >= 1 && g.a <= 31 && g.a + P.k >= 32 && (P.rec_n == 0 || P.rec_lo + P.rec_n <= 31)
-	       && g.up <= g.a && g.sh_x >= 0 && g.sh_x <= 31 && g.sh_y1 >= 0 && g.sh_y1 <= 32 && (P.rec_n == 0 || P.rec_lo + P.rec_n == P.bf_shift - 9) && P.R <= g.up;
-	return g;
-}
+__host__ __device__ __forceinline__ Dec3 dec3_geom(const KParams &P) { return dec3_make(P.k, P.bf_shift, P.R, P.F, P.rec_lo, P.rec_n); }
 
 #define FS32_EMPTY 0xffffffffu
 __device__ __forceinline__ uint32_t fs32_slot(uint32_t bitoff, uint32_t mask) { return ((bitoff * 0x9E3779B1u) >> 12 ^ bitoff) & mask; }
diff --git a/bfc_amd/csrc/bfcg_internal.h b/bfc_amd/csrc/bfcg_internal.h
--- a/bfc_amd/csrc/bfcg_internal.h
+++ b/bfc_amd/csrc/bfcg_internal.h
@@ -62,6 +62,7 @@
 	int b3fm;
 	int l2_big;
 	int b3_cold;
+	int rec2_b3;
 };
 
 struct BatchBufs {
@@ -97,6 +98,7 @@
 int bloom_lds_bytes(const KParams &P);
 bool bloom3fm_geometry_ok(const KParams &P);
 bool bloom3_geometry_ok(const KParams &P);
+BFCG_LOCAL bool stage_b_rec2_b3(const KParams &P, const BatchBufs &B);
 BFCG_LOCAL bool scatter2_big_ok(const KParams &P);
 hipError_t set_bloom_lds_attr(const KParams &P);
 void run_query(const KParams &P, const uint8_t *seq, int64_t n_pos, const void *bloom, uint8_t *flags, hipStream_t st);
diff --git a/bfc_amd/csrc/bfcg_kernels.hip b/bfc_amd/csrc/bfcg_kernels.hip
--- a/bfc_amd/csrc/bfcg_kernels.hip
+++ b/bfc_amd/csrc/bfcg_kernels.hip
@@ -542,6 +542,8 @@
 	}
 	__syncthreads();
 	const uint32_t n_in = n_live;
+	const Dec3 D3 = dec3_geom(P);
+	const bool b3 = RW == 3 && P.rec2_b3;
 	for (uint32_t pos = threadIdx.x; pos < n_in; pos += BT) {
 		RecW<RW> rec;
 #pragma unroll
@@ -551,6 +553,7 @@
 		else if constexpr (FAST2) b = (rec.d[0] >> P.R) & (uint32_t)(nb2 - 1);
 		else { uint64_t y0, y1; uint32_t idx; bool hi; Rec<RW>::unpack(rec, RG, imp, y0, y1, idx, hi); b = fine_id<W>(P, y0, y1) & (uint32_t)(nb2 - 1); }
 		const uint64_t dst = (uint32_t)(pos + gdelta[b]);
+		if (b3) rec3_b3_pack(D3, imp, rec.d[0], rec.d[1]);
 		rec_store<RW>(out + dst * RW, rec);
 	}
 }
@@ -1956,6 +1959,15 @@
 	       && P.R <= up && up >= 1 && up <= 31 && a >= up + 18 && io + 32 <= 128;
 }
 bool bloom3_geometry_ok(const KParams &P) { return bfcg_rec_dwords(P.k, P.rec_n) == 3 && P.n_hashes == 4 && P.R <= 8 && bloom_fast3(P); }
+static bool batch_takes_bloom3(const KParams &P, const BatchBufs &B)
+{
+	return !(P.filter_mode && B.bloom_hi) && P.seg && B.seg_tab && (B.stream_out || B.ho) && bfcg_rec_dwords(P.k, P.rec_n) == 3 && P.b3 && (P.b3_cold || !P.dedupe);
+}
+bool stage_b_rec2_b3(const KParams &P, const BatchBufs &B)
+{
+	const char *e = getenv("BFCG_REC2_B3");
+	return P.F2 > 0 && batch_takes_bloom3(P, B) && dec3_make(P.k, P.bf_shift, P.R, P.F, P.rec_lo, P.rec_n).b3_ok && !(e && atoi(e) == 0);
+}
 bool scatter2_big_ok(const KParams &P) { return bfcg_rec_dwords(P.k, P.rec_n) == 3 && scatter2_fast(P); }
 
 static dim3 seg_grid(const KParams &P, uint32_t n_fine, uint32_t bt)
@@ -2022,7 +2034,7 @@
 	} else if (P.seg && B.seg_tab && (B.stream_out || B.ho)) {
 		A.stream_out = B.stream_out; A.seg_tab = B.seg_tab; A.table = nullptr; A.agg_out = nullptr;
 		A.ho = B.ho; A.ho_stride = B.ho_stride; A.ho_cur = B.ho_cur; A.ho_mark = B.ho_stride ? B.ho_mark + (size_t)B.ho_page * B.ho_mark_stride : nullptr;
-		if (RW == 3 && P.b3 && (P.b3_cold || !P.dedupe)) run_bloom3(P, A, nfine, (size_t)bloom_lds_bytes(P), st);
+		if (batch_takes_bloom3(P, B)) run_bloom3(P, A, nfine, (size_t)bloom_lds_bytes(P), st);
 		else launch_bloom<W, RW>(!h4 ? BV_SEG_ANYH : RW == 3 && bloom_fast3(P) ? BV_SEG_F3 : BV_SEG, P, A, nfine, st);
 	} else if (B.stream && B.stream_out && !P.track && h4) {
 		A.stream_out = B.stream_out;
@@ -2047,10 +2059,12 @@
 }
 
 template <typename W, int RW>
-static void run_stage_b_t(const KParams &P, const BatchBufs &B, const uint32_t *in1, const uint32_t *seg_beg, const uint32_t *seg_end, int n_seg,
+static void run_stage_b_t(const KParams &P_in, const BatchBufs &B, const uint32_t *in1, const uint32_t *seg_beg, const uint32_t *seg_end, int n_seg,
                           int segs_per_bucket, const uint32_t *row_base, const uint32_t *bucket_start, uint64_t n_rec_bound, hipStream_t st, hipEvent_t *ev)
 {
+	KParams P = P_in;
 	const int nfine = (n_seg / segs_per_bucket) << P.F2;
+	P.rec2_b3 = stage_b_rec2_b3(P_in, B);
 	const auto [fine_recs, fine_start] = run_level2_t<W, RW>(P, B, in1, seg_beg, seg_end, n_seg, segs_per_bucket, row_base, bucket_start, n_rec_bound, st);
 	if (ev) hipEventRecord(ev[3], st);
 	BloomArgs A = run_bloom_t<W, RW>(P, B, fine_recs, fine_start, nfine, st);
diff --git a/bfc_amd/csrc/bfcg_kmers.hip b/bfc_amd/csrc/bfcg_kmers.hip
--- a/bfc_amd/csrc/bfcg_kmers.hip
+++ b/bfc_amd/csrc/bfcg_kmers.hip
@@ -7,6 +7,7 @@
 #include "bfcg_internal.h"
 #include "bfc_host.h"
 #include "bfcg_kdec.h"
+#include "kmer_dev.h"
 
 namespace {
 
@@ -346,6 +347,48 @@
 	return Y0 == Z0 && Y1 == Z1 ? 0 : -1;
 }
 
+static int rec2_geom(const int geom[5], bfcg::Dec3 &D)
+{
+	const int k = geom[0], bf_shift = geom[1], R = geom[2], F2 = geom[3], rec_n = geom[4];
+	if (k < 1 || k > 63 || bf_shift < 10 || R < 0 || R > 8 || F2 < 0 || rec_n < 0 || bf_shift - 9 - R < F2 || bfcg_rec_dwords(k, rec_n) != 3) return -1;
+	D = bfcg::dec3_make(k, bf_shift, R, bf_shift - 9 - R, R + F2, rec_n);
+	return D.b3_ok ? 0 : -1;
+}
+extern "C" int bfcg_rec2_b3_pack_host(const int geom[5], uint64_t n, const uint32_t *imp, const uint32_t *in, uint32_t *out)
+{
+	bfcg::Dec3 D;
+	if (rec2_geom(geom, D) != 0) return -1;
+	for (uint64_t i = 0; i < n; ++i) {
+		uint32_t d0 = in[3 * i], d1 = in[3 * i + 1];
+		bfcg::rec3_b3_pack(D, imp[i], d0, d1);
+		out[3 * i] = d0; out[3 * i + 1] = d1; out[3 * i + 2] = in[3 * i + 2];
+	}
+	return 0;
+}
+extern "C" int bfcg_rec2_addr_host(const int geom[5], int b3, uint64_t n, const uint32_t *imp, const uint32_t *recs, uint32_t *addr)
+{
+	bfcg::Dec3 D;
+	if (rec2_geom(geom, D) != 0) return -1;
+	for (uint64_t i = 0; i < n; ++i) addr[i] = b3 ? bfcg::rec3_b3_addr(D, recs[3 * i], recs[3 * i + 1]) : bfcg::rec3_addr(D, imp[i], recs[3 * i], recs[3 * i + 1]);
+	return 0;
+}
+extern "C" int bfcg_rec2_entry_host(const int geom[5], int b3, uint64_t n, const uint32_t *recs, uint64_t *entry)
+{
+	bfcg::Dec3 D;
+	if (rec2_geom(geom, D) != 0) return -1;
+	for (uint64_t i = 0; i < n; ++i) entry[i] = b3 ? bfcg::rec3_b3_entry(D, recs[3 * i], recs[3 * i + 1]) : bfcg::rec3_entry(D, recs[3 * i], recs[3 * i + 1]);
+	return 0;
+}
+extern "C" int bfcg_rec2_entry_unpack_host(const int geom[5], uint64_t n, const uint64_t *region, const uint64_t *entry, uint64_t *y, uint8_t *high)
+{
+	bfcg::Dec3 D;
+	if (rec2_geom(geom, D) != 0) return -1;
+	const int k = geom[0], lo = geom[2] < k ? geom[2] : k, top = k < geom[1] - 9 ? k : geom[1] - 9;
+	const bfcg::SegGeom G = {k, lo, top > lo ? top : lo};
+	for (uint64_t i = 0; i < n; ++i) { bfcg::seg_unpack(G, region[i], entry[i] >> 1, y[2 * i], y[2 * i + 1]); high[i] = (uint8_t)(entry[i] & 1); }
+	return 0;
+}
+
 extern "C" void bfcg_kmer_2str(int k, const uint64_t y[2], char *buf)
 {
 	for (int l = 0; l < k; ++l) buf[k - 1 - l] = "ACGT"[(y[1] >> l & 1) << 1 | (y[0] >> l & 1)];
diff --git a/bfc_amd/csrc/kmer_dev.h b/bfc_amd/csrc/kmer_dev.h
--- a/bfc_amd/csrc/kmer_dev.h
+++ b/bfc_amd/csrc/kmer_dev.h
@@ -144,6 +144,74 @@
 }
 __host__ __device__ __forceinline__ uint32_t seg_home(uint64_t id) { return (uint32_t)((id * 0x9E3779B97F4A7C15ULL) >> 38); }
 
+struct Dec3 { int ok, a, lo, n, up, sh_x, R, sh_flag, sh_y1, k, s_hx, b3_ok; uint32_t lowmask, rmask, mk32, mask_a, upmask, hxmask, emask_lo, emask_hi; };
+__host__ __device__ __forceinline__ Dec3 dec3_make(int k, int bf_shift, int R, int F, int rec_lo, int rec_n)
+{
+	Dec3 g;
+	g.k = k; g.a = k - rec_n; g.lo = rec_lo; g.n = rec_n; g.up = rec_n ? rec_lo : bf_shift - 9; g.sh_x = k - (bf_shift - 9);
+	g.R = R; g.sh_flag = g.a + k - 32; g.sh_y1 = k - F;
+	g.lowmask = rec_n ? (1u << (rec_lo & 31)) - 1u : 0xffffffffu; g.rmask = (1u << R) - 1u; g.mk32 = k >= 32 ? 0xffffffffu : (1u << k) - 1u;
+	g.ok = k >= bf_shift - 9 && bf_shift + 9 <= 2 * k && g.a >= 1 && g.a <= 31 && g.a + k >= 32 && (rec_n == 0 || rec_lo + rec_n <= 31)
+	       && g.up <= g.a && g.sh_x >= 0 && g.sh_x <= 31 && g.sh_y1 >= 0 && g.sh_y1 <= 32 && (rec_n == 0 || rec_lo + rec_n == bf_shift - 9) && R <= g.up;
+	g.mask_a = g.a >= 1 && g.a <= 31 ? (1u << g.a) - 1u : 0xffffffffu;
+	const int n_hx = g.sh_x >= 0 && g.sh_x < 18 ? 18 - g.sh_x : 0;
+	g.s_hx = 2 * k - F + 1;
+	g.b3_ok = g.ok && R <= 8 && g.s_hx >= 1 && g.s_hx <= 63 && g.s_hx + n_hx <= 63;
+	g.upmask = g.sh_x >= 0 && g.sh_x < 18 ? (1u << g.sh_x) - 1u : 0x3ffffu;
+	g.hxmask = (1u << n_hx) - 1u;
+	const unsigned long long em = g.s_hx >= 1 && g.s_hx <= 63 ? (1ULL << g.s_hx) - 1ULL : ~0ULL;
+	g.emask_lo = (uint32_t)em; g.emask_hi = (uint32_t)(em >> 32);
+	return g;
+}
+__host__ __device__ __forceinline__ uint32_t rec3_bits(uint32_t hi, uint32_t lo, int s)
+{
+#if defined(__HIP_DEVICE_COMPILE__)
+	return __builtin_amdgcn_alignbit(hi, lo, (uint32_t)s);
+#else
+	return (uint32_t)((((uint64_t)hi << 32) | lo) >> s);
+#endif
+}
+__host__ __device__ __forceinline__ uint32_t rec3_addr_pack(uint32_t bl, uint32_t hh)
+{
+	uint32_t h2 = (hh >> 9) & 511u;
+	h2 |= (uint32_t)((h2 & 31u) == 0);
+	return bl | ((hh & 511u) << 8) | (h2 << 17);
+}
+__host__ __device__ __forceinline__ uint32_t rec3_x(const Dec3 &D, uint32_t imp, uint32_t d0, uint32_t d1)
+{
+	const uint32_t y0d = d0 & D.mask_a, upper = y0d >> D.up;
+	const uint32_t y0lo = D.n ? (y0d & D.lowmask) | (imp << D.lo) | (upper << (D.lo + D.n)) : y0d;
+	const uint32_t y1lo = rec3_bits(d1, d0, D.a) & D.mk32;
+	return (y0lo - y1lo) ^ y1lo;
+}
+__host__ __device__ __forceinline__ uint32_t rec3_addr(const Dec3 &D, uint32_t imp, uint32_t d0, uint32_t d1)
+{
+	const uint32_t y0d = d0 & D.mask_a;
+	return rec3_addr_pack(y0d & D.rmask, (y0d >> D.up) | (rec3_x(D, imp, d0, d1) << D.sh_x));
+}
+__host__ __device__ __forceinline__ unsigned long long rec3_entry(const Dec3 &D, uint32_t d0, uint32_t d1)
+{
+	const unsigned long long AA = d0 | ((unsigned long long)d1 << 32);
+	const unsigned long long y1 = (AA >> D.a) & ((1ULL << D.k) - 1);
+	const uint32_t y0d = d0 & D.mask_a;
+	const unsigned long long id = (unsigned long long)((y0d & D.rmask) | ((y0d >> D.up) << D.R)) | (y1 << D.sh_y1);
+	return (id << 1) | (unsigned long long)((d1 >> D.sh_flag) & 1u);
+}
+__host__ __device__ __forceinline__ void rec3_b3_pack(const Dec3 &D, uint32_t imp, uint32_t &d0, uint32_t &d1)
+{
+	const unsigned long long e = rec3_entry(D, d0, d1) | ((unsigned long long)(rec3_x(D, imp, d0, d1) & D.hxmask) << D.s_hx);
+	d0 = (uint32_t)e; d1 = (uint32_t)(e >> 32);
+}
+__host__ __device__ __forceinline__ uint32_t rec3_b3_addr(const Dec3 &D, uint32_t d0, uint32_t d1)
+{
+	const uint32_t hx = (uint32_t)((d0 | ((unsigned long long)d1 << 32)) >> D.s_hx);
+	return rec3_addr_pack((d0 >> 1) & D.rmask, ((d0 >> (1 + D.R)) & D.upmask) | (hx << D.sh_x));
+}
+__host__ __device__ __forceinline__ unsigned long long rec3_b3_entry(const Dec3 &D, uint32_t d0, uint32_t d1)
+{
+	return (d0 & D.emask_lo) | ((unsigned long long)(d1 & D.emask_hi) << 32);
+}
+
 struct BloomAddr {
 	uint64_t blk;
 	uint32_t h1, h2;
diff --git a/include/bfc_gpu.h b/include/bfc_gpu.h
--- a/include/bfc_gpu.h
+++ b/include/bfc_gpu.h
@@ -192,6 +192,10 @@
 int   bfcg_kmers_list(bfcg_kmers_t *t, int min_cnt, int min_diff, uint32_t sub_lo, uint32_t sub_hi, uint64_t *y, uint16_t *cnt_high, uint64_t cap, uint64_t *n);
 float bfcg_kmers_last_ms(bfcg_kmers_t *t);
 int   bfcg_kmer_decode_host(int k, int l_pre, uint32_t sub, uint64_t slot, uint64_t y[2]);
+int   bfcg_rec2_b3_pack_host(const int geom[5], uint64_t n, const uint32_t *imp, const uint32_t *in, uint32_t *out);
+int   bfcg_rec2_addr_host(const int geom[5], int b3, uint64_t n, const uint32_t *imp, const uint32_t *recs, uint32_t *addr);
+int   bfcg_rec2_entry_host(const int geom[5], int b3, uint64_t n, const uint32_t *recs, uint64_t *entry);
+int   bfcg_rec2_entry_unpack_host(const int geom[5], uint64_t n, const uint64_t *region, const uint64_t *entry, uint64_t *y, uint8_t *high);
 void  bfcg_kmer_2str(int k, const uint64_t y[2], char *buf);
 uint64_t bfcg_kmers_format(int k, const uint64_t *y, const uint16_t *cnt_high, uint64_t n, char *buf);
 uint64_t bfcg_kmers_format_sizes(const uint32_t *sizes, uint64_t n, char *buf);
```

New measurement: 41000, median of 2. About the same (+0.8%).
